# alpa-projects/alpa

Hardware: AMD Instinct MI355X
Metric: model_tflops_aggregate (higher is better)
Workload: dtype bf16; 1 GPU; model=GPT-2.6B, hidden=2560, layers=32, heads=32, vocab=51200, global_batch=32, seq_len=1024, num_micro_batches=1, parallelism=dp1, hip_graph=True

## Files before the change

alpa_amd/ops/__init__.py:

```python
from __future__ import annotations

import functools
import math
from typing import List, NamedTuple, Optional

import torch

from . import reference as ref
from ._backend import hip_ops, hip_ops_available, use_hip

__all__ = [
    "layer_norm", "add_layer_norm", "bias_gelu", "add_layer_norm_fp8",
    "bias_gelu_fp8", "flash_attention",
    "flash_attention_qkv", "flash_attention_decode", "decode_attn_ok",
    "DECODE_ATTN_CHUNK", "softmax_cross_entropy",
    "softmax_cross_entropy_partial", "softmax_cross_entropy_combine",
    "softmax_cross_entropy_shard_bwd", "vocab_ce_fused_ok", "fused_adamw",
    "multi_tensor_sumsq",
    "hip_ops_available", "MoERouting", "moe_top2_route", "moe_dispatch",
    "moe_combine", "moe_fused_ok",
]


class _LayerNorm(torch.autograd.Function):

    @staticmethod
    def forward(ctx, x, weight, bias, eps):
        x = x.contiguous()
        if use_hip(x):
            y, mean, rstd = hip_ops().layer_norm_fwd(x, weight, bias, eps)
        else:
            y, mean, rstd = ref.layer_norm_fwd(x, weight, bias, eps)
        ctx.save_for_backward(x, weight, mean, rstd)
        return y

    @staticmethod
    def backward(ctx, dy):
        x, weight, mean, rstd = ctx.saved_tensors
        if use_hip(x):
            dx, dw, db = hip_ops().layer_norm_bwd(dy.contiguous(), x, weight,
                                                  mean, rstd)
        else:
            dx, dw, db = ref.layer_norm_bwd(dy, x, weight, mean, rstd)
        return dx, dw.to(weight.dtype), db.to(weight.dtype), None


def layer_norm(x: torch.Tensor, weight: torch.Tensor, bias: torch.Tensor,
               eps: float = 1e-5) -> torch.Tensor:
    return _LayerNorm.apply(x, weight, bias, eps)


class _AddLayerNorm(torch.autograd.Function):

    @staticmethod
    def forward(ctx, a, delta, weight, bias, eps):
        a = a.contiguous()
        delta = delta.contiguous() if delta is not None else None
        if use_hip(a):
            h, y, mean, rstd = hip_ops().add_layer_norm_fwd(
                a, delta, weight, bias, eps)
        else:
            h = a + delta if delta is not None else a
            y, mean, rstd = ref.layer_norm_fwd(h, weight, bias, eps)
        ctx.save_for_backward(h, weight, mean, rstd)
        ctx.has_delta = delta is not None
        return h, y

    @staticmethod
    def backward(ctx, dh, dy):
        h, weight, mean, rstd = ctx.saved_tensors
        dy = dy.contiguous()
        dhc = dh.contiguous() if dh is not None else None
        if use_hip(h):
            dx, dw, db = hip_ops().add_layer_norm_bwd(dy, dhc, h, weight,
                                                      mean, rstd)
        else:
            dx, dw, db = ref.layer_norm_bwd(dy, h, weight, mean, rstd)
            if dhc is not None:
                dx = dx + dhc
        g2 = dx if ctx.has_delta else None
        return dx, g2, dw.to(weight.dtype), db.to(weight.dtype), None


def add_layer_norm(a: torch.Tensor, delta, weight: torch.Tensor,
                   bias: torch.Tensor, eps: float = 1e-5):
    if delta is None:
        return a, _LayerNorm.apply(a, weight, bias, eps)
    return _AddLayerNorm.apply(a, delta, weight, bias, eps)


class _BiasGelu(torch.autograd.Function):

    @staticmethod
    def forward(ctx, x, bias):
        x = x.contiguous()
        ctx.save_for_backward(x, bias)
        if use_hip(x):
            return hip_ops().bias_gelu_fwd(x, bias)
        return ref.bias_gelu_fwd(x, bias)

    @staticmethod
    def backward(ctx, dy):
        x, bias = ctx.saved_tensors
        if use_hip(x):
            dx, db = hip_ops().bias_gelu_bwd(dy.contiguous(), x, bias)
        else:
            dx, db = ref.bias_gelu_bwd(dy, x, bias)
        return dx, db.to(bias.dtype)


def bias_gelu(x: torch.Tensor, bias: torch.Tensor) -> torch.Tensor:
    return _BiasGelu.apply(x, bias)


@torch.no_grad()
def bias_gelu_fp8(x: torch.Tensor, bias: torch.Tensor, scale: torch.Tensor):
    x = x.contiguous()
    if use_hip(x):
        return tuple(hip_ops().bias_gelu_fp8(x, bias, scale))
    return ref.bias_gelu_fp8(x, bias, scale)


ADD_LAYER_NORM_FP8_MAX_H = 4096


@torch.no_grad()
def add_layer_norm_fp8(a: torch.Tensor, delta, weight: torch.Tensor,
                       bias: torch.Tensor, eps: float, scale: torch.Tensor):
    a = a.contiguous()
    delta = delta.contiguous() if delta is not None else None
    if use_hip(a):
        return tuple(hip_ops().add_layer_norm_fp8(a, delta, weight, bias,
                                                  eps, scale))
    return ref.add_layer_norm_fp8(a, delta, weight, bias, eps, scale)


class _BiasAdd(torch.autograd.Function):

    @staticmethod
    def forward(ctx, x, bias):
        ctx.feat = bias.shape[-1]
        ctx.bias_dtype = bias.dtype
        return x + bias

    @staticmethod
    def backward(ctx, g):
        if use_hip(g) and g.dtype == torch.bfloat16:
            db = hip_ops().colsum_bf16(
                g.contiguous().reshape(-1, ctx.feat))
            db = db.to(ctx.bias_dtype)
        else:
            dims = tuple(range(g.dim() - 1))
            db = g.sum(dim=dims).to(ctx.bias_dtype)
        return g, db


def bias_add(x: torch.Tensor, bias: torch.Tensor) -> torch.Tensor:
    return _BiasAdd.apply(x, bias)


class _LinearBias(torch.autograd.Function):

    @staticmethod
    def forward(ctx, x, w, bias):
        shape = x.shape
        x2 = x.reshape(-1, shape[-1])
        y = torch.addmm(bias, x2, w.t())
        ctx.save_for_backward(x2, w)
        ctx.bias_dtype = bias.dtype
        return y.reshape(*shape[:-1], w.shape[0])

    @staticmethod
    def backward(ctx, g):
        x2, w = ctx.saved_tensors
        g2 = g.reshape(-1, g.shape[-1]).contiguous()
        dx = (g2 @ w).reshape(*g.shape[:-1], w.shape[1])
        dw = g2.t() @ x2
        if use_hip(g2) and g2.dtype == torch.bfloat16:
            db = hip_ops().colsum_bf16(g2).to(ctx.bias_dtype)
        else:
            db = g2.sum(0).to(ctx.bias_dtype)
        return dx, dw, db


def linear_bias(x: torch.Tensor, w: torch.Tensor,
                bias: torch.Tensor) -> torch.Tensor:
    return _LinearBias.apply(x, w, bias)


class _FlashAttention(torch.autograd.Function):

    @staticmethod
    def forward(ctx, q, k, v, causal, scale, alibi=None):
        if scale is None:
            scale = 1.0 / math.sqrt(q.shape[-1])
        if use_hip(q):
            if q.shape[-1] > 128:
                assert alibi is None, "alibi requires head_dim <= 128"
                if q.shape[2] >= 128 and q.shape[-1] <= 256:
                    o, lse = hip_ops().attn_fwd(q, k, v, causal, scale,
                                                None)
                else:
                    o, lse = hip_ops().attn_fwd_blocked(q, k, v, causal,
                                                        scale)
            else:
                o, lse = hip_ops().attn_fwd(q, k, v, causal, scale, alibi)
        else:
            o, lse = ref.attention_fwd(q, k, v, causal, scale, alibi)
        ctx.save_for_backward(q, k, v, o, lse)
        ctx.causal = causal
        ctx.scale = scale
        ctx.alibi = alibi
        return o

    @staticmethod
    def backward(ctx, do):
        q, k, v, o, lse = ctx.saved_tensors
        if use_hip(q):
            if q.shape[-1] > 128:
                dq, dk, dv = hip_ops().attn_bwd_blocked(
                    do.contiguous(), q, k, v, o, lse, ctx.causal, ctx.scale)
            else:
                dq, dk, dv = hip_ops().attn_bwd(
                    do.contiguous(), q, k, v, o, lse, ctx.causal, ctx.scale,
                    ctx.alibi)
        else:
            dq, dk, dv = ref.attention_bwd(do, q, k, v, o, lse, ctx.causal,
                                           ctx.scale, ctx.alibi)
        return dq, dk, dv, None, None, None


def flash_attention(q: torch.Tensor, k: torch.Tensor, v: torch.Tensor,
                    causal: bool = True,
                    scale: Optional[float] = None,
                    alibi_slopes: Optional[torch.Tensor] = None
                    ) -> torch.Tensor:
    if q.shape[2] == 1 and not causal and _decode_attn_routed(q, k, v) and \
            not (torch.is_grad_enabled() and
                 (q.requires_grad or k.requires_grad or v.requires_grad)):
        if scale is None:
            scale = 1.0 / math.sqrt(q.shape[-1])
        return hip_ops().attn_decode(q, k, v, scale, alibi_slopes, None)[0]
    return _FlashAttention.apply(q, k, v, causal, scale, alibi_slopes)


_DECODE_ATTN_CHUNK = {64: 128, 128: 128, 256: 128}


def DECODE_ATTN_CHUNK(head_dim: int) -> int:
    for dp in sorted(_DECODE_ATTN_CHUNK):
        if head_dim <= dp:
            return _DECODE_ATTN_CHUNK[dp]
    raise ValueError(f"head_dim {head_dim} is above 256")


def _rows_aligned16(t: torch.Tensor) -> bool:
    return t.data_ptr() % 16 == 0 and all(
        t.shape[i] <= 1 or t.stride(i) % 8 == 0 for i in range(3))


def decode_attn_ok(q: torch.Tensor, k: torch.Tensor, v: torch.Tensor) -> bool:
    for t in (q, k, v):
        if not (t.is_cuda and t.dtype == torch.bfloat16 and t.dim() == 4
                and t.stride(3) == 1):
            return False
    D = q.shape[3]
    if q.shape[2] != 1 or D % 16 != 0 or not 16 <= D <= 256:
        return False
    if k.shape != v.shape or k.shape[:2] != q.shape[:2] or k.shape[3] != D \
            or q.shape[0] * q.shape[1] > 65535:
        return False
    if not all(_rows_aligned16(t) for t in (q, k, v)):
        return False
    return use_hip(q)


def _decode_attn_routed(q, k, v) -> bool:
    from ..global_env import global_config
    if global_config.decode_attention in ("0", False):
        return False
    return decode_attn_ok(q, k, v)


@torch.no_grad()
def flash_attention_decode(q: torch.Tensor, k: torch.Tensor, v: torch.Tensor,
                           kv_lens: Optional[torch.Tensor] = None,
                           scale: Optional[float] = None,
                           alibi_slopes: Optional[torch.Tensor] = None
                           ) -> torch.Tensor:
    if scale is None:
        scale = 1.0 / math.sqrt(q.shape[-1])
    lens = None if kv_lens is None else kv_lens.to(dtype=torch.int32)
    if decode_attn_ok(q, k, v):
        return hip_ops().attn_decode(
            q, k, v, scale, alibi_slopes,
            None if lens is None else lens.contiguous())[0]
    o, _ = ref.attention_fwd(q, k, v, False, scale, alibi_slopes, lens)
    return o


@torch.no_grad()
def flash_attention_varlen(q: torch.Tensor, k: torch.Tensor,
                           v: torch.Tensor, kv_lens: torch.Tensor,
                           scale: Optional[float] = None,
                           alibi_slopes: Optional[torch.Tensor] = None
                           ) -> torch.Tensor:
    if scale is None:
        scale = 1.0 / math.sqrt(q.shape[-1])
    lens = kv_lens.to(dtype=torch.int32)
    if use_hip(q):
        if q.shape[2] == 1 and _decode_attn_routed(q, k, v):
            return hip_ops().attn_decode(q, k, v, scale, alibi_slopes,
                                         lens.contiguous())[0]
        if q.shape[-1] > 128:
            raise NotImplementedError(
                "varlen attention with more than one query row, or with "
                "the decode kernel off, requires head_dim <= 128")
        o, _ = hip_ops().attn_fwd(q.contiguous(), k.contiguous(),
                                  v.contiguous(), False, scale,
                                  alibi_slopes, lens.contiguous())
        return o
    o, _ = ref.attention_fwd(q, k, v, False, scale, alibi_slopes, lens)
    return o


def _qkv_views(qkv: torch.Tensor, num_heads: int):
    B, S, F = qkv.shape
    qkv5 = qkv.view(B, S, num_heads, 3, F // (3 * num_heads))
    return tuple(qkv5[:, :, :, i].permute(0, 2, 1, 3) for i in range(3))


class _FlashAttentionQKV(torch.autograd.Function):

    @staticmethod
    def forward(ctx, qkv, num_heads, causal, scale):
        B, S, F = qkv.shape
        h = num_heads
        d = F // (3 * h)
        if scale is None:
            scale = 1.0 / math.sqrt(d)
        q, k, v = _qkv_views(qkv, h)
        if use_hip(qkv):
            o_buf = torch.empty(B, S, h * d, dtype=qkv.dtype,
                                device=qkv.device)
            o_view = o_buf.view(B, S, h, d).permute(0, 2, 1, 3)
            lse = torch.empty(B, h, S, dtype=torch.float32,
                              device=qkv.device)
            hip_ops().attn_fwd_out(q, k, v, o_view, lse, causal, scale)
        else:
            o4, lse = ref.attention_fwd(q.contiguous(), k.contiguous(),
                                        v.contiguous(), causal, scale)
            o_buf = o4.permute(0, 2, 1, 3).reshape(B, S, h * d)
        ctx.save_for_backward(qkv, o_buf, lse)
        ctx.meta = (num_heads, causal, scale)
        return o_buf

    @staticmethod
    def backward(ctx, do):
        qkv, o_buf, lse = ctx.saved_tensors
        h, causal, scale = ctx.meta
        B, S, F = qkv.shape
        d = F // (3 * h)
        q, k, v = _qkv_views(qkv, h)
        do4 = do.view(B, S, h, d).permute(0, 2, 1, 3)
        o4 = o_buf.view(B, S, h, d).permute(0, 2, 1, 3)
        dqkv = torch.empty_like(qkv)
        dq_v, dk_v, dv_v = _qkv_views(dqkv, h)
        if use_hip(qkv):
            hip_ops().attn_bwd_out(do4, q, k, v, o4, lse, dq_v, dk_v, dv_v,
                                   causal, scale)
        else:
            dq, dk, dv = ref.attention_bwd(
                do4.contiguous(), q.contiguous(), k.contiguous(),
                v.contiguous(), o4.contiguous(), lse, causal, scale)
            dq_v.copy_(dq)
            dk_v.copy_(dk)
            dv_v.copy_(dv)
        return dqkv, None, None, None


def flash_attention_qkv(qkv: torch.Tensor, num_heads: int,
                        causal: bool = True,
                        scale: Optional[float] = None) -> torch.Tensor:
    return _FlashAttentionQKV.apply(qkv, num_heads, causal, scale)


class _SoftmaxCrossEntropy(torch.autograd.Function):

    @staticmethod
    def forward(ctx, logits, targets):
        logits = logits.contiguous()
        if use_hip(logits):
            loss, lse = hip_ops().cross_entropy_fwd(logits, targets)
        else:
            loss, lse = ref.softmax_cross_entropy_fwd(logits, targets)
        ctx.save_for_backward(logits, targets, lse)
        return loss

    @staticmethod
    def backward(ctx, dloss):
        logits, targets, lse = ctx.saved_tensors
        if use_hip(logits):
            dlogits = hip_ops().cross_entropy_bwd(dloss.contiguous(), logits,
                                                  targets, lse)
        else:
            dlogits = ref.softmax_cross_entropy_bwd(dloss, logits, targets, lse)
        return dlogits, None


def softmax_cross_entropy(logits: torch.Tensor,
                          targets: torch.Tensor) -> torch.Tensor:
    return _SoftmaxCrossEntropy.apply(logits, targets)




def vocab_ce_fused_ok(logits: torch.Tensor) -> bool:
    if not (logits.is_cuda and logits.dtype == torch.bfloat16):
        return False
    if logits.dim() != 2 or not logits.is_contiguous():
        return False
    if logits.shape[-1] < 8 or logits.shape[-1] % 8 != 0 or \
            logits.data_ptr() % 16 != 0:
        return False
    return use_hip(logits)


@torch.no_grad()
def softmax_cross_entropy_partial(logits: torch.Tensor,
                                  targets: torch.Tensor,
                                  vocab_start: int) -> torch.Tensor:
    if use_hip(logits):
        return hip_ops().cross_entropy_partial_fwd(
            logits.contiguous(), targets.contiguous(), int(vocab_start))
    return ref.softmax_cross_entropy_partial(logits, targets,
                                             int(vocab_start))


@torch.no_grad()
def softmax_cross_entropy_combine(stats: torch.Tensor):
    return ref.softmax_cross_entropy_combine(stats)


@torch.no_grad()
def softmax_cross_entropy_shard_bwd(dloss: torch.Tensor,
                                    logits: torch.Tensor,
                                    targets: torch.Tensor, lse: torch.Tensor,
                                    vocab_start: int) -> torch.Tensor:
    if use_hip(logits):
        return hip_ops().cross_entropy_shard_bwd(
            dloss.contiguous(), logits.contiguous(), targets.contiguous(),
            lse, int(vocab_start))
    return ref.softmax_cross_entropy_shard_bwd(dloss, logits, targets, lse,
                                               int(vocab_start))


_ADAM_CHUNK = 16384
_ADAM_TABLE_CACHE: dict = {}


def _upload_tables(rows, dev):
    n = len(rows)
    descs = torch.tensor(rows, dtype=torch.int64).reshape(n, 6)
    counts = [(r[4] + _ADAM_CHUNK - 1) // _ADAM_CHUNK for r in rows]
    tensor_idx = torch.repeat_interleave(
        torch.arange(n, dtype=torch.int32),
        torch.tensor(counts, dtype=torch.int64))
    chunk_idx = torch.cat([torch.arange(c, dtype=torch.int32)
                           for c in counts])
    chunks = torch.stack([tensor_idx, chunk_idx], dim=1).contiguous()
    return descs.to(dev), chunks.to(dev)


def _adam_tables(params, grads, exp_avgs, exp_avg_sqs):
    key = tuple((p.data_ptr(), g.data_ptr(), m.data_ptr(), v.data_ptr(),
                 p.numel(), p.dtype)
                for p, g, m, v in zip(params, grads, exp_avgs, exp_avg_sqs))
    hit = _ADAM_TABLE_CACHE.get(key)
    if hit is not None:
        return hit
    rows = []
    for p, g, m, v in zip(params, grads, exp_avgs, exp_avg_sqs):
        assert p.is_contiguous() and g.is_contiguous()
        assert m.dtype == torch.float32 and v.dtype == torch.float32
        assert p.dtype == g.dtype and p.dtype in (torch.bfloat16,
                                                  torch.float32)
        rows.append((p.data_ptr(), g.data_ptr(), m.data_ptr(), v.data_ptr(),
                     p.numel(), 1 if p.dtype == torch.bfloat16 else 0))
    tbl = _upload_tables(rows, params[0].device)
    _ADAM_TABLE_CACHE[key] = tbl
    return tbl


_SUMSQ_TABLE_CACHE: dict = {}


def _sumsq_tables(tensors):
    key = tuple((t.data_ptr(), t.numel(), t.dtype) for t in tensors)
    hit = _SUMSQ_TABLE_CACHE.get(key)
    if hit is not None:
        return hit
    rows = []
    for t in tensors:
        assert t.is_contiguous()
        assert t.dtype in (torch.bfloat16, torch.float32)
        rows.append((0, t.data_ptr(), 0, 0, t.numel(),
                     1 if t.dtype == torch.bfloat16 else 0))
    dev = tensors[0].device
    descs, chunks = _upload_tables(rows, dev)
    partials = torch.empty(chunks.shape[0], dtype=torch.float32, device=dev)
    tbl = (descs, chunks, partials)
    _SUMSQ_TABLE_CACHE[key] = tbl
    return tbl


@torch.no_grad()
def multi_tensor_sumsq(tensors: List[torch.Tensor]) -> torch.Tensor:
    tensors = [t for t in tensors if t.numel() > 0]
    if not tensors:
        raise ValueError("multi_tensor_sumsq needs at least one element")
    if use_hip(tensors[0]):
        descs, chunks, partials = _sumsq_tables(tensors)
        out = torch.empty(1, dtype=torch.float32, device=tensors[0].device)
        hip_ops().multi_tensor_sumsq_raw(descs, chunks, partials, out)
        return out
    return ref.multi_tensor_sumsq(tensors)


@torch.no_grad()
def fused_adamw(params: List[torch.Tensor], grads: List[torch.Tensor],
                exp_avgs: List[torch.Tensor], exp_avg_sqs: List[torch.Tensor],
                step: int, lr: float, beta1: float = 0.9, beta2: float = 0.95,
                eps: float = 1e-8, weight_decay: float = 0.0,
                grad_scale: float = 1.0,
                grad_sumsq: Optional[torch.Tensor] = None,
                max_grad_norm: Optional[float] = None) -> None:
    if (grad_sumsq is None) != (max_grad_norm is None):
        raise ValueError(
            "grad_sumsq and max_grad_norm must be given together")
    if max_grad_norm is not None and not max_grad_norm > 0:
        raise ValueError(f"max_grad_norm must be > 0, got {max_grad_norm}")
    if not params:
        return
    if use_hip(params[0]):
        descs, chunks = _adam_tables(params, grads, exp_avgs, exp_avg_sqs)
        hip_ops().adamw_step_raw(descs, chunks, step, lr, beta1, beta2, eps,
                                 weight_decay, grad_scale, grad_sumsq,
                                 max_grad_norm or 0.0)
    else:
        ref.adamw_step(params, grads, exp_avgs, exp_avg_sqs, step, lr, beta1,
                       beta2, eps, weight_decay, grad_scale, grad_sumsq,
                       max_grad_norm)




class MoERouting(NamedTuple):
    w1: torch.Tensor
    w2: torch.Tensor
    idx1: torch.Tensor
    idx2: torch.Tensor
    slot1: torch.Tensor
    slot2: torch.Tensor
    src: torch.Tensor
    aux_loss: torch.Tensor


class _MoeTop2Route(torch.autograd.Function):

    @staticmethod
    def forward(ctx, logits, capacity):
        logits = logits.contiguous()
        if use_hip(logits):
            outs = hip_ops().moe_route_fwd(logits, capacity)
        else:
            outs = ref.moe_top2_route(logits, capacity)
        w1, w2, idx1, idx2, slot1, slot2, src, aux, count1 = outs
        ctx.save_for_backward(logits, idx1, idx2, w1, w2, count1)
        ctx.mark_non_differentiable(idx1, idx2, slot1, slot2, src)
        return w1, w2, idx1, idx2, slot1, slot2, src, aux

    @staticmethod
    def backward(ctx, dw1, dw2, _i1, _i2, _s1, _s2, _src, daux):
        logits, idx1, idx2, w1, w2, count1 = ctx.saved_tensors
        if use_hip(logits):
            return hip_ops().moe_route_bwd(
                logits, idx1, idx2, w1, w2, count1, dw1.float().contiguous(),
                dw2.float().contiguous(), daux.float().contiguous()), None
        return ref.moe_top2_route_bwd(logits, idx1, idx2, w1, w2, count1,
                                      dw1, dw2, daux), None


def moe_top2_route(logits: torch.Tensor, capacity: int) -> MoERouting:
    return MoERouting(*_MoeTop2Route.apply(logits, int(capacity)))


class _MoeDispatch(torch.autograd.Function):

    @staticmethod
    def forward(ctx, x, src, slot1, slot2):
        x = x.contiguous()
        ctx.save_for_backward(slot1, slot2)
        if use_hip(x):
            return hip_ops().moe_dispatch(x, src)
        return ref.moe_dispatch(x, src)

    @staticmethod
    def backward(ctx, g):
        slot1, slot2 = ctx.saved_tensors
        if use_hip(g):
            dx = hip_ops().moe_combine(g.contiguous(), None, None, slot1,
                                       slot2)
        else:
            dx = ref.moe_dispatch_bwd(g, slot1, slot2)
        return dx, None, None, None


def moe_dispatch(x: torch.Tensor, routing: MoERouting) -> torch.Tensor:
    return _MoeDispatch.apply(x, routing.src, routing.slot1, routing.slot2)


class _MoeCombine(torch.autograd.Function):

    @staticmethod
    def forward(ctx, y, w1, w2, slot1, slot2, src):
        y = y.contiguous()
        ctx.save_for_backward(y, w1, w2, slot1, slot2, src)
        if use_hip(y):
            return hip_ops().moe_combine(y, w1.float().contiguous(),
                                         w2.float().contiguous(), slot1,
                                         slot2)
        return ref.moe_combine(y, w1, w2, slot1, slot2)

    @staticmethod
    def backward(ctx, dout):
        y, w1, w2, slot1, slot2, src = ctx.saved_tensors
        if use_hip(y):
            dout = dout.contiguous()
            dy = hip_ops().moe_dispatch(dout, src, slot1,
                                        w1.float().contiguous(),
                                        w2.float().contiguous())
            dw1, dw2 = hip_ops().moe_combine_dw(dout, y, slot1, slot2)
            dw1, dw2 = dw1.to(w1.dtype), dw2.to(w2.dtype)
        else:
            dy, dw1, dw2 = ref.moe_combine_bwd(dout, y, w1, w2, slot1,
                                               slot2, src)
        return dy, dw1, dw2, None, None, None


def moe_combine(y: torch.Tensor, routing: MoERouting) -> torch.Tensor:
    return _MoeCombine.apply(y, routing.w1, routing.w2, routing.slot1,
                             routing.slot2, routing.src)


def moe_fused_ok(x: torch.Tensor, num_experts: int,
                 capacity: Optional[int] = None) -> bool:
    if not (x.is_cuda and x.dtype == torch.bfloat16):
        return False
    if x.shape[-1] < 8 or x.shape[-1] % 8 != 0 or \
            not 2 <= num_experts <= 128:
        return False
    if capacity is not None and num_experts * capacity >= 2 ** 31:
        return False
    return use_hip(x)



def _skinny_mt(M: int) -> int:
    MT = 4
    while MT < M:
        MT *= 2
    return MT


def _skinny_legal_splits(K: int, MT: int) -> List[int]:
    q = K // 64
    return [s for s in range(1, q + 1)
            if q % s == 0 and (K // 8 // s) * 16 * MT <= 65536]


@functools.lru_cache(maxsize=None)
def _skinny_splits(N: int, K: int, M: int) -> Optional[int]:
    lds_ok = _skinny_legal_splits(K, _skinny_mt(M))
    if not lds_ok:
        return None
    for s in sorted(lds_ok, reverse=True):
        if K // 8 // s >= 16 and (N // 64) * s >= 1024:
            return s
    for s in lds_ok:
        if (N // 64) * s >= 2560:
            return s
    return lds_ok[-1]


def _skinny_cache(module, weight: torch.Tensor, fp8: bool):
    key = (weight._version, fp8)
    cached = getattr(module, "_skinny_pack", None)
    if cached is not None and cached[0] == key:
        return cached[1], cached[2]
    N, K = weight.shape
    with torch.no_grad():
        w = weight.contiguous()
        if fp8:
            amax = w.abs().amax().float().clamp_min(1e-12)
            scale = (amax / 448.0).reshape(1)
            q = (w.float() / scale).clamp(-448.0, 448.0).to(
                torch.float8_e4m3fn)
            wp = q.view(torch.uint8).view(N, K // 8, 8) \
                .permute(1, 0, 2).contiguous()
        else:
            scale = None
            wp = w.view(N, K // 8, 8).permute(1, 0, 2).contiguous()
    module._skinny_pack = (key, wp, scale)
    return wp, scale


def skinny_ok(x: torch.Tensor, weight: torch.Tensor, module=None) -> bool:
    from ..global_env import global_config
    mode = global_config.skinny_gemm
    if mode in ("0", False) or torch.is_grad_enabled():
        return False
    if not (x.is_cuda and x.dtype == torch.bfloat16):
        return False
    if torch.cuda.is_current_stream_capturing() and \
            getattr(module, "_skinny_pack", None) is None:
        return False
    N, K = weight.shape
    if mode == "auto" and (K > 6144 and N > 6144):
        fp8 = (global_config.fp8_gemm and
               not getattr(module, "_fp8_exclude", False))
        if not fp8:
            return False
    m = x.numel() // x.shape[-1]
    return (m <= 8 and N % 64 == 0 and K % 64 == 0
            and _skinny_splits(N, K, m) is not None)


_SKINNY_TUNED = {}


def _skinny_tune(wp, x2, scale, N, K, MT):
    key = (N, K, MT, scale is not None)
    got = _SKINNY_TUNED.get(key)
    if got is not None:
        return got
    legal = _skinny_legal_splits(K, MT)
    cands = sorted({
        s for s in (
            next((c for c in reversed(legal)
                  if K // 8 // c >= 16 and (N // 64) * c >= 1024), None),
            next((c for c in legal if (N // 64) * c >= 2560), None),
            next((c for c in legal if K // 8 // c <= 32), None),
            legal[-1]) if s is not None})
    if len(cands) == 1:
        _SKINNY_TUNED[key] = cands[0]
        return cands[0]
    best, best_t = cands[0], float("inf")
    for c in cands:
        hip_ops().skinny_gemm(wp, x2, scale, None, N, K, c)
        t0 = torch.cuda.Event(True)
        t1 = torch.cuda.Event(True)
        t0.record()
        for _ in range(10):
            hip_ops().skinny_gemm(wp, x2, scale, None, N, K, c)
        t1.record()
        t1.synchronize()
        dt = t0.elapsed_time(t1)
        if dt < best_t:
            best, best_t = c, dt
    _SKINNY_TUNED[key] = best
    return best


def skinny_linear(x: torch.Tensor, weight: torch.Tensor,
                  bias: Optional[torch.Tensor], module) -> torch.Tensor:
    from ..global_env import global_config
    fp8 = (global_config.fp8_gemm and
           not getattr(module, "_fp8_exclude", False))
    wp, scale = _skinny_cache(module, weight, fp8)
    N, K = weight.shape
    shape = x.shape
    x2 = x.reshape(-1, K).contiguous()
    b = bias.contiguous() if bias is not None else None
    MT = _skinny_mt(x2.shape[0])
    if torch.cuda.is_current_stream_capturing():
        splits = _SKINNY_TUNED.get((N, K, MT, scale is not None)) \
            or _skinny_splits(N, K, x2.shape[0])
    else:
        splits = _skinny_tune(wp, x2, scale, N, K, MT)
    y = hip_ops().skinny_gemm(wp, x2, scale, b, N, K, splits)
    return y.reshape(*shape[:-1], N)
```

alpa_amd/ops/csrc/bias_gelu.hip:

```cpp
#include "common.h"
#include "fused_math.h"
#include "launchers.h"

__device__ __forceinline__ float gelu_grad_f(float x) {
  const float k = 0.7978845608028654f;
  float x2 = x * x;
  float sg = gelu_sigmoid(x);
  return sg + 2.0f * x * sg * (1.0f - sg) * k *
                  (1.0f + 3.f * 0.044715f * x2);
}

__global__ void bias_gelu_fwd_kernel(const short* __restrict__ x,
                                     const short* __restrict__ bias,
                                     short* __restrict__ y, int64_t total,
                                     int F) {
  int64_t idx = ((int64_t)blockIdx.x * blockDim.x + threadIdx.x) * 8;
  int64_t stride = (int64_t)gridDim.x * blockDim.x * 8;
  for (; idx < total; idx += stride) {
    bf16x8 v = *reinterpret_cast<const bf16x8*>(x + idx);
    bf16x8 bv = *reinterpret_cast<const bf16x8*>(bias + (idx % F));
    bf16x8 o;
#pragma unroll
    for (int j = 0; j < 8; ++j) o[j] = f2bf(gelu_f(bf2f(v[j]) + bf2f(bv[j])));
    *reinterpret_cast<bf16x8*>(y + idx) = o;
  }
}

__global__ void bias_gelu_bwd_dx_kernel(const short* __restrict__ dy,
                                        const short* __restrict__ x,
                                        const short* __restrict__ bias,
                                        short* __restrict__ dx, int64_t total,
                                        int F) {
  int64_t idx = ((int64_t)blockIdx.x * blockDim.x + threadIdx.x) * 8;
  int64_t stride = (int64_t)gridDim.x * blockDim.x * 8;
  for (; idx < total; idx += stride) {
    bf16x8 dv = *reinterpret_cast<const bf16x8*>(dy + idx);
    bf16x8 xv = *reinterpret_cast<const bf16x8*>(x + idx);
    bf16x8 bv = *reinterpret_cast<const bf16x8*>(bias + (idx % F));
    bf16x8 o;
#pragma unroll
    for (int j = 0; j < 8; ++j) {
      float z = bf2f(xv[j]) + bf2f(bv[j]);
      o[j] = f2bf(bf2f(dv[j]) * gelu_grad_f(z));
    }
    *reinterpret_cast<bf16x8*>(dx + idx) = o;
  }
}

__global__ void bias_grad_partial_kernel(const short* __restrict__ dx,
                                         float* __restrict__ part, int64_t N,
                                         int F) {
  const int col8 = (blockIdx.x * blockDim.x + threadIdx.x) * 8;
  const int p = blockIdx.y;
  const int P = gridDim.y;
  const int64_t r0 = (int64_t)p * N / P, r1 = (int64_t)(p + 1) * N / P;
  if (col8 + 8 <= F) {
    float s[8] = {0.f, 0.f, 0.f, 0.f, 0.f, 0.f, 0.f, 0.f};
    for (int64_t row = r0; row < r1; ++row) {
      bf16x8 v = *reinterpret_cast<const bf16x8*>(dx + row * F + col8);
#pragma unroll
      for (int j = 0; j < 8; ++j) s[j] += bf2f(v[j]);
    }
#pragma unroll
    for (int j = 0; j < 8; ++j) part[(int64_t)p * F + col8 + j] = s[j];
  } else if (col8 < F) {
    for (int c = col8; c < F; ++c) {
      float s = 0.f;
      for (int64_t row = r0; row < r1; ++row) s += bf2f(dx[row * F + c]);
      part[(int64_t)p * F + c] = s;
    }
  }
}

extern "C" {

hipError_t launch_bias_gelu_fwd(const void* x, const void* bias, void* y,
                                int64_t N, int64_t F, hipStream_t stream) {
  int64_t total = N * F;
  int blocks = (int)min((int64_t)2048, ceil_div(total, 256 * 8));
  bias_gelu_fwd_kernel<<<dim3(blocks), dim3(256), 0, stream>>>(
      (const short*)x, (const short*)bias, (short*)y, total, (int)F);
  return hipGetLastError();
}

hipError_t launch_colsum_partial(const void* t, float* part, int64_t N,
                                 int64_t F, int P, hipStream_t stream) {
  dim3 grid((uint32_t)ceil_div(F, 256 * 8), P);
  bias_grad_partial_kernel<<<grid, dim3(256), 0, stream>>>(
      (const short*)t, part, N, (int)F);
  return hipGetLastError();
}

hipError_t launch_bias_gelu_bwd(const void* dy, const void* x,
                                const void* bias, void* dx, float* db_part,
                                int64_t N, int64_t F, int P,
                                hipStream_t stream) {
  int64_t total = N * F;
  int blocks = (int)min((int64_t)2048, ceil_div(total, 256 * 8));
  bias_gelu_bwd_dx_kernel<<<dim3(blocks), dim3(256), 0, stream>>>(
      (const short*)dy, (const short*)x, (const short*)bias, (short*)dx,
      total, (int)F);
  dim3 grid((uint32_t)ceil_div(F, 256 * 8), P);
  bias_grad_partial_kernel<<<grid, dim3(256), 0, stream>>>(
      (const short*)dx, db_part, N, (int)F);
  return hipGetLastError();
}

}
```

alpa_amd/ops/csrc/bindings.cpp:

```cpp
#include <torch/extension.h>

#include <ATen/ATen.h>
#include <c10/hip/HIPStream.h>
#include <hip/hip_runtime.h>

#include <vector>
#include <algorithm>
#include <array>
#include <utility>

#include "launchers.h"

#define HIP_OK(expr)                                                       \
  do {                                                                     \
    hipError_t _e = (expr);                                                \
    TORCH_CHECK(_e == hipSuccess, "HIP error: ", hipGetErrorString(_e));   \
  } while (0)

namespace {

hipStream_t cur_stream() {
  return c10::hip::getCurrentHIPStream().stream();
}


const char* dtype_name(at::ScalarType dtype) {
  switch (dtype) {
    case at::kBFloat16: return "bf16";
    case at::kFloat: return "fp32";
    case at::kInt: return "int32";
    case at::kLong: return "int64";
    default: return c10::toString(dtype);
  }
}

void check_device(const at::Tensor& t, const char* name,
                  const at::Tensor& first) {
  TORCH_CHECK(t.is_cuda(), name, " must be on GPU");
  TORCH_CHECK(t.device() == first.device(), name, " is on ", t.device(),
              " but the first operand is on ", first.device());
}

void check_typed(const at::Tensor& t, const char* name, at::ScalarType dtype,
                 const at::Tensor& first) {
  check_device(t, name, first);
  TORCH_CHECK(t.scalar_type() == dtype, name, " must be ", dtype_name(dtype));
}

void check_vec(const at::Tensor& t, const char* name, at::ScalarType dtype,
               int64_t n, const at::Tensor& first) {
  check_typed(t, name, dtype, first);
  TORCH_CHECK(t.is_contiguous(), name, " must be contiguous");
  TORCH_CHECK(t.numel() == n, name, " must have ", n, " elements, got ",
              t.numel());
}

std::pair<int64_t, int64_t> check_rows(const at::Tensor& t, const char* name,
                                       int64_t m, const at::Tensor& first) {
  check_typed(t, name, at::kBFloat16, first);
  TORCH_CHECK(t.is_contiguous(), name, " must be contiguous");
  TORCH_CHECK(t.dim() >= 1, name, " must have a feature dimension");
  const int64_t W = t.size(-1);
  TORCH_CHECK(W > 0 && W % m == 0, name,
              ": the last dimension must be a positive multiple of ", m,
              ", got ", W);
  return {t.numel() / W, W};
}

void check_like(const at::Tensor& t, const char* name, const at::Tensor& ref,
                const char* ref_name) {
  check_typed(t, name, at::kBFloat16, ref);
  TORCH_CHECK(t.is_contiguous(), name, " must be contiguous");
  TORCH_CHECK(t.sizes() == ref.sizes(), name, " must have the shape of ",
              ref_name);
}

void check_bhsd(const at::Tensor& t, const char* name, int64_t B, int64_t H,
                int64_t S, int64_t D, const at::Tensor& first) {
  check_typed(t, name, at::kBFloat16, first);
  TORCH_CHECK(t.dim() == 4, name, " must be 4-D [B,H,S,D]");
  TORCH_CHECK(t.stride(3) == 1, name, " head-dim must be contiguous");
  const int64_t want[4] = {B, H, S, D};
  for (int i = 0; i < 4; ++i)
    TORCH_CHECK(want[i] < 0 || t.size(i) == want[i], name, " must have size ",
                want[i], " in dimension ", i, ", got ", t.size(i));
}

void check_rows_aligned16(const at::Tensor& t, const char* name) {
  TORCH_CHECK(reinterpret_cast<uintptr_t>(t.const_data_ptr()) % 16 == 0, name,
              " must be 16-byte aligned");
  for (int i = 0; i < 3; ++i)
    TORCH_CHECK(t.size(i) <= 1 || t.stride(i) % 8 == 0, name,
                ": the stride of dimension ", i,
                " must be a multiple of 8 elements, got ", t.stride(i));
}

std::pair<int64_t, int64_t> check_aligned_rows(const at::Tensor& t,
                                               const char* name,
                                               const at::Tensor& first) {
  auto dims = check_rows(t, name, 8, first);
  TORCH_CHECK(t.dim() == 2, name, " must be 2-D");
  TORCH_CHECK(reinterpret_cast<uintptr_t>(t.const_data_ptr()) % 16 == 0, name,
              " must be 16-byte aligned");
  return dims;
}

int stripes_for(int64_t N, int64_t cols, int64_t chunk_cols) {
  int64_t chunks = std::max<int64_t>(1, cols / chunk_cols);
  int64_t p = std::max<int64_t>(64, 2048 / chunks);
  return (int)std::min<int64_t>({p, N, 512});
}


std::vector<at::Tensor> layer_norm_fwd(const at::Tensor& x,
                                       const at::Tensor& w,
                                       const at::Tensor& b, double eps) {
  auto [N, H] = check_rows(x, "x", 8, x);
  check_vec(w, "w", at::kBFloat16, H, x);
  check_vec(b, "b", at::kBFloat16, H, x);
  auto y = at::empty_like(x);
  auto f32 = x.options().dtype(at::kFloat);
  auto mean = at::empty({N}, f32);
  auto rstd = at::empty({N}, f32);
  HIP_OK(launch_layer_norm_fwd(x.const_data_ptr(), w.const_data_ptr(),
                               b.const_data_ptr(), y.mutable_data_ptr(),
                               (float*)mean.mutable_data_ptr(),
                               (float*)rstd.mutable_data_ptr(), N, H,
                               (float)eps, cur_stream()));
  return {y, mean, rstd};
}

std::pair<at::Tensor, at::Tensor> layer_norm_dwdb(const at::Tensor& dy,
                                                  const at::Tensor& x,
                                                  const at::Tensor& mean,
                                                  const at::Tensor& rstd,
                                                  int64_t N, int64_t H) {
  auto f32 = x.options().dtype(at::kFloat);
  auto dw = at::empty({H}, f32);
  auto db = at::empty({H}, f32);
  const int kStripes = stripes_for(N, H, 256);
  auto dw_part = at::empty({kStripes, H}, f32);
  auto db_part = at::empty({kStripes, H}, f32);
  HIP_OK(launch_layer_norm_bwd_dwdb(
      dy.const_data_ptr(), x.const_data_ptr(),
      (const float*)mean.const_data_ptr(),
      (const float*)rstd.const_data_ptr(),
      (float*)dw_part.mutable_data_ptr(), (float*)db_part.mutable_data_ptr(),
      N, H, kStripes, cur_stream()));
  at::sum_out(dw, dw_part, {0});
  at::sum_out(db, db_part, {0});
  return {dw, db};
}

std::vector<at::Tensor> layer_norm_bwd(const at::Tensor& dy,
                                       const at::Tensor& x,
                                       const at::Tensor& w,
                                       const at::Tensor& mean,
                                       const at::Tensor& rstd) {
  auto [N, H] = check_rows(x, "x", 8, x);
  check_like(dy, "dy", x, "x");
  check_vec(w, "w", at::kBFloat16, H, x);
  check_vec(mean, "mean", at::kFloat, N, x);
  check_vec(rstd, "rstd", at::kFloat, N, x);
  auto dx = at::empty_like(x);
  HIP_OK(launch_layer_norm_bwd_dx(
      dy.const_data_ptr(), nullptr, x.const_data_ptr(), w.const_data_ptr(),
      (const float*)mean.const_data_ptr(), (const float*)rstd.const_data_ptr(),
      dx.mutable_data_ptr(), N, H, cur_stream()));
  auto [dw, db] = layer_norm_dwdb(dy, x, mean, rstd, N, H);
  return {dx, dw, db};
}


std::vector<at::Tensor> add_layer_norm_fwd(const at::Tensor& a,
                                           const c10::optional<at::Tensor>& b,
                                           const at::Tensor& w,
                                           const at::Tensor& bias,
                                           double eps) {
  auto [N, H] = check_rows(a, "a", 8, a);
  if (b.has_value()) check_like(*b, "b", a, "a");
  check_vec(w, "w", at::kBFloat16, H, a);
  check_vec(bias, "bias", at::kBFloat16, H, a);
  auto h = at::empty_like(a);
  auto y = at::empty_like(a);
  auto f32 = a.options().dtype(at::kFloat);
  auto mean = at::empty({N}, f32);
  auto rstd = at::empty({N}, f32);
  const void* bp = b.has_value() ? b->const_data_ptr() : nullptr;
  HIP_OK(launch_add_layer_norm_fwd(
      a.const_data_ptr(), bp, w.const_data_ptr(), bias.const_data_ptr(),
      h.mutable_data_ptr(), y.mutable_data_ptr(),
      (float*)mean.mutable_data_ptr(), (float*)rstd.mutable_data_ptr(), N,
      H, (float)eps, cur_stream()));
  return {h, y, mean, rstd};
}

std::vector<at::Tensor> add_layer_norm_bwd(
    const at::Tensor& dy, const c10::optional<at::Tensor>& dh,
    const at::Tensor& h, const at::Tensor& w, const at::Tensor& mean,
    const at::Tensor& rstd) {
  auto [N, H] = check_rows(h, "h", 8, h);
  check_like(dy, "dy", h, "h");
  if (dh.has_value()) check_like(*dh, "dh", h, "h");
  check_vec(w, "w", at::kBFloat16, H, h);
  check_vec(mean, "mean", at::kFloat, N, h);
  check_vec(rstd, "rstd", at::kFloat, N, h);
  auto dx = at::empty_like(h);
  const void* dhp = dh.has_value() ? dh->const_data_ptr() : nullptr;
  HIP_OK(launch_layer_norm_bwd_dx(
      dy.const_data_ptr(), dhp, h.const_data_ptr(), w.const_data_ptr(),
      (const float*)mean.const_data_ptr(),
      (const float*)rstd.const_data_ptr(), dx.mutable_data_ptr(), N, H,
      cur_stream()));
  auto [dw, db] = layer_norm_dwdb(dy, h, mean, rstd, N, H);
  return {dx, dw, db};
}


at::Tensor bias_gelu_fwd(const at::Tensor& x, const at::Tensor& bias) {
  auto [N, F] = check_rows(x, "x", 8, x);
  check_vec(bias, "bias", at::kBFloat16, F, x);
  auto y = at::empty_like(x);
  HIP_OK(launch_bias_gelu_fwd(x.const_data_ptr(), bias.const_data_ptr(),
                              y.mutable_data_ptr(), N, F, cur_stream()));
  return y;
}

std::vector<at::Tensor> bias_gelu_bwd(const at::Tensor& dy,
                                      const at::Tensor& x,
                                      const at::Tensor& bias) {
  auto [N, F] = check_rows(x, "x", 8, x);
  check_like(dy, "dy", x, "x");
  check_vec(bias, "bias", at::kBFloat16, F, x);
  auto dx = at::empty_like(x);
  auto f32 = x.options().dtype(at::kFloat);
  const int kStripes = stripes_for(N, F, 2048);
  auto db = at::empty({F}, f32);
  auto db_part = at::empty({kStripes, F}, f32);
  HIP_OK(launch_bias_gelu_bwd(dy.const_data_ptr(), x.const_data_ptr(),
                              bias.const_data_ptr(), dx.mutable_data_ptr(),
                              (float*)db_part.mutable_data_ptr(), N, F,
                              kStripes, cur_stream()));
  at::sum_out(db, db_part, {0});
  return {dx, db};
}

at::Tensor colsum_bf16(const at::Tensor& t) {
  auto [N, F] = check_rows(t, "t", 1, t);
  auto f32 = t.options().dtype(at::kFloat);
  const int kStripes = stripes_for(N, F, 2048);
  auto part = at::empty({kStripes, F}, f32);
  auto out = at::empty({F}, f32);
  HIP_OK(launch_colsum_partial(t.const_data_ptr(),
                               (float*)part.mutable_data_ptr(), N, F,
                               kStripes, cur_stream()));
  at::sum_out(out, part, {0});
  return out;
}


at::Tensor skinny_gemm(const at::Tensor& wp, const at::Tensor& x,
                       const c10::optional<at::Tensor>& wscale,
                       const c10::optional<at::Tensor>& bias,
                       int64_t N, int64_t K, int64_t splits) {
  TORCH_CHECK(N > 0 && N % 64 == 0, "N must be a positive multiple of 64");
  TORCH_CHECK(K > 0 && K % 64 == 0, "K must be a positive multiple of 64");
  const bool fp8 = wscale.has_value();
  if (fp8) {
    check_device(wp, "wp", wp);
    TORCH_CHECK(wp.element_size() == 1,
                "wp must hold one-byte elements when wscale is given");
    TORCH_CHECK(wp.is_contiguous() && wp.numel() == N * K,
                "wp must be contiguous with N*K elements");
    check_vec(*wscale, "wscale", at::kFloat, 1, wp);
  } else {
    check_vec(wp, "wp", at::kBFloat16, N * K, wp);
  }
  if (bias.has_value()) check_vec(*bias, "bias", at::kBFloat16, N, wp);
  auto [M, Kx] = check_rows(x, "x", 64, wp);
  TORCH_CHECK(x.dim() == 2 && Kx == K, "x must be [M, K]");
  TORCH_CHECK(M >= 1 && M <= 64, "skinny path is for M <= 64");
  int64_t MT = 4;
  while (MT < M) MT *= 2;
  TORCH_CHECK(splits >= 1 && (K / 64) % splits == 0 &&
                  (K / 8 / splits) * 16 * MT <= 65536,
              "splits must divide K/64 and leave (K/8/splits)*16*MT <= 65536");
  at::Tensor xp = x;
  if (MT != M) {
    xp = at::zeros({MT, K}, x.options());
    xp.narrow(0, 0, M).copy_(x);
  }
  auto part = at::empty({splits, MT, N}, x.options().dtype(at::kFloat));
  auto y = at::empty({M, N}, x.options());
  HIP_OK(launch_skinny_gemm(
      wp.const_data_ptr(), xp.const_data_ptr(),
      (float*)part.mutable_data_ptr(),
      bias.has_value() ? bias->const_data_ptr() : nullptr,
      y.mutable_data_ptr(),
      fp8 ? (const float*)wscale->const_data_ptr() : nullptr, M, MT, N, K,
      (int)splits, fp8 ? 1 : 0, cur_stream()));
  return y;
}


void adamw_step_raw(const at::Tensor& descs, const at::Tensor& chunks,
                    int64_t step, double lr, double beta1, double beta2,
                    double eps, double weight_decay, double grad_scale,
                    const c10::optional<at::Tensor>& grad_sumsq,
                    double max_grad_norm) {
  TORCH_CHECK(descs.dim() == 2 && descs.size(1) == 6, "descs must be [n, 6]");
  TORCH_CHECK(chunks.dim() == 2 && chunks.size(1) == 2,
              "chunks must be [m, 2]");
  check_vec(descs, "descs", at::kLong, descs.numel(), descs);
  check_vec(chunks, "chunks", at::kInt, chunks.numel(), descs);
  const float* sumsq = nullptr;
  if (grad_sumsq.has_value()) {
    check_vec(*grad_sumsq, "grad_sumsq", at::kFloat, 1, descs);
    TORCH_CHECK(max_grad_norm > 0, "max_grad_norm must be positive");
    sumsq = (const float*)grad_sumsq->const_data_ptr();
  }
  HIP_OK(launch_adamw(descs.const_data_ptr(), chunks.const_data_ptr(),
                      (int)chunks.size(0), (float)lr, (float)beta1,
                      (float)beta2, (float)eps, (float)weight_decay,
                      (float)grad_scale, (int)step, sumsq,
                      (float)max_grad_norm, cur_stream()));
}

void multi_tensor_sumsq_raw(const at::Tensor& descs, const at::Tensor& chunks,
                            at::Tensor& partials, at::Tensor& out) {
  TORCH_CHECK(descs.dim() == 2 && descs.size(1) == 6, "descs must be [n, 6]");
  TORCH_CHECK(chunks.dim() == 2 && chunks.size(1) == 2,
              "chunks must be [m, 2]");
  check_vec(descs, "descs", at::kLong, descs.numel(), descs);
  check_vec(chunks, "chunks", at::kInt, chunks.numel(), descs);
  int64_t n = chunks.size(0);
  check_typed(partials, "partials", at::kFloat, descs);
  TORCH_CHECK(partials.is_contiguous() && partials.numel() >= n,
              "partials must be contiguous with at least num_chunks elements");
  check_vec(out, "out", at::kFloat, 1, descs);
  HIP_OK(launch_multi_tensor_sumsq(
      descs.const_data_ptr(), chunks.const_data_ptr(), (int)n,
      (float*)partials.mutable_data_ptr(), (float*)out.mutable_data_ptr(),
      cur_stream()));
}


std::vector<at::Tensor> cross_entropy_fwd(const at::Tensor& logits,
                                          const at::Tensor& targets) {
  auto [N, V] = check_rows(logits, "logits", 8, logits);
  check_vec(targets, "targets", at::kLong, N, logits);
  auto f32 = logits.options().dtype(at::kFloat);
  auto loss = at::empty({N}, f32);
  auto lse = at::empty({N}, f32);
  HIP_OK(launch_ce_fwd(logits.const_data_ptr(),
                       (const int64_t*)targets.const_data_ptr(),
                       (float*)loss.mutable_data_ptr(),
                       (float*)lse.mutable_data_ptr(), N, V, cur_stream()));
  return {loss, lse};
}

at::Tensor cross_entropy_bwd(const at::Tensor& dloss, const at::Tensor& logits,
                             const at::Tensor& targets,
                             const at::Tensor& lse) {
  auto [N, V] = check_rows(logits, "logits", 8, logits);
  check_vec(targets, "targets", at::kLong, N, logits);
  check_vec(lse, "lse", at::kFloat, N, logits);
  check_device(dloss, "dloss", logits);
  TORCH_CHECK(dloss.numel() == N, "dloss must have ", N, " elements, got ",
              dloss.numel());
  auto dlogits = at::empty_like(logits);
  auto dl = dloss.to(at::kFloat).contiguous();
  HIP_OK(launch_ce_bwd((const float*)dl.const_data_ptr(), logits.const_data_ptr(),
                       (const int64_t*)targets.const_data_ptr(),
                       (const float*)lse.const_data_ptr(),
                       dlogits.mutable_data_ptr(), N, V, 0, cur_stream()));
  return dlogits;
}

at::Tensor cross_entropy_partial_fwd(const at::Tensor& logits,
                                     const at::Tensor& targets,
                                     int64_t vocab_start) {
  auto [N, V] = check_aligned_rows(logits, "logits", logits);
  check_vec(targets, "targets", at::kLong, N, logits);
  TORCH_CHECK(vocab_start >= 0, "vocab_start must be >= 0");
  auto stats = at::empty({3, N}, logits.options().dtype(at::kFloat));
  HIP_OK(launch_ce_partial_fwd(logits.const_data_ptr(),
                               (const int64_t*)targets.const_data_ptr(),
                               (float*)stats.mutable_data_ptr(), N, V,
                               vocab_start, cur_stream()));
  return stats;
}

at::Tensor cross_entropy_shard_bwd(const at::Tensor& dloss,
                                   const at::Tensor& logits,
                                   const at::Tensor& targets,
                                   const at::Tensor& lse,
                                   int64_t vocab_start) {
  auto [N, V] = check_aligned_rows(logits, "logits", logits);
  check_vec(targets, "targets", at::kLong, N, logits);
  TORCH_CHECK(vocab_start >= 0, "vocab_start must be >= 0");
  check_vec(lse, "lse", at::kFloat, N, logits);
  check_device(dloss, "dloss", logits);
  TORCH_CHECK(dloss.numel() == N, "dloss must have ", N, " elements, got ",
              dloss.numel());
  auto dlogits = at::empty_like(logits);
  auto dl = dloss.to(at::kFloat).contiguous();
  HIP_OK(launch_ce_bwd((const float*)dl.const_data_ptr(),
                       logits.const_data_ptr(),
                       (const int64_t*)targets.const_data_ptr(),
                       (const float*)lse.const_data_ptr(),
                       dlogits.mutable_data_ptr(), N, V, vocab_start,
                       cur_stream()));
  return dlogits;
}



template <typename... T>
std::array<int64_t, 3 * sizeof...(T)> bhs_strides(const T&... t) {
  std::array<int64_t, 3 * sizeof...(T)> s;
  int64_t* p = s.data();
  ((*p++ = t.stride(0), *p++ = t.stride(1), *p++ = t.stride(2)), ...);
  return s;
}

bool given(const c10::optional<at::Tensor>& t) {
  return t.has_value() && t->defined();
}

const void* opt_ptr(const c10::optional<at::Tensor>& t) {
  return given(t) ? t->const_data_ptr() : nullptr;
}

void check_attn_inputs(const at::Tensor& q, const at::Tensor& k,
                       const at::Tensor& v,
                       const c10::optional<at::Tensor>& alibi,
                       const c10::optional<at::Tensor>& kv_lens,
                       int64_t max_D) {
  check_bhsd(q, "q", -1, -1, -1, -1, q);
  const int64_t B = q.size(0), H = q.size(1), D = q.size(3);
  check_bhsd(k, "k", B, H, -1, D, q);
  check_bhsd(v, "v", B, H, k.size(2), D, q);
  TORCH_CHECK(D > 0 && D % 16 == 0 && D <= max_D,
              "head_dim must be a multiple of 16 up to ", max_D, ", got ", D);
  TORCH_CHECK(D <= 128 || !(given(alibi) || given(kv_lens)),
              "alibi and kv_lens need head_dim <= 128, got ", D);
  if (given(alibi)) check_vec(*alibi, "alibi", at::kFloat, H, q);
  if (given(kv_lens)) check_vec(*kv_lens, "kv_lens", at::kInt, B, q);
}

at::Tensor attn_fwd_out(const at::Tensor& q, const at::Tensor& k,
                        const at::Tensor& v, at::Tensor o, at::Tensor lse,
                        bool causal, double scale,
                        const c10::optional<at::Tensor>& alibi =
                            c10::nullopt,
                        const c10::optional<at::Tensor>& kv_lens =
                            c10::nullopt) {
  check_attn_inputs(q, k, v, alibi, kv_lens, 256);
  int64_t B = q.size(0), H = q.size(1), S = q.size(2), D = q.size(3);
  int64_t Skv = k.size(2);
  check_bhsd(o, "o", B, H, S, D, q);
  check_vec(lse, "lse", at::kFloat, B * H * S, q);
  const auto strides = bhs_strides(q, k, v, o);
  HIP_OK(launch_attn_fwd(q.const_data_ptr(), k.const_data_ptr(),
                         v.const_data_ptr(), o.mutable_data_ptr(),
                         (float*)lse.mutable_data_ptr(), B, H, S, Skv, D,
                         (float)scale, causal ? 1 : 0,
                         (const float*)opt_ptr(alibi),
                         (const int*)opt_ptr(kv_lens), strides.data(),
                         cur_stream()));
  return o;
}

std::vector<at::Tensor> attn_fwd(const at::Tensor& q, const at::Tensor& k,
                                 const at::Tensor& v, bool causal,
                                 double scale,
                                 const c10::optional<at::Tensor>& alibi =
                                     c10::nullopt,
                                 const c10::optional<at::Tensor>& kv_lens =
                                     c10::nullopt) {
  check_attn_inputs(q, k, v, alibi, kv_lens, 256);
  int64_t B = q.size(0), H = q.size(1), S = q.size(2);
  auto o = at::empty_like(q.contiguous());
  auto lse = at::empty({B, H, S}, q.options().dtype(at::kFloat));
  attn_fwd_out(q, k, v, o, lse, causal, scale, alibi, kv_lens);
  return {o, lse};
}

std::vector<at::Tensor> attn_decode(const at::Tensor& q, const at::Tensor& k,
                                    const at::Tensor& v, double scale,
                                    const c10::optional<at::Tensor>& alibi =
                                        c10::nullopt,
                                    const c10::optional<at::Tensor>& kv_lens =
                                        c10::nullopt) {
  check_bhsd(q, "q", -1, -1, -1, -1, q);
  const int64_t B = q.size(0), H = q.size(1), D = q.size(3);
  TORCH_CHECK(q.size(2) == 1, "q must hold one query row per head, got ",
              q.size(2));
  check_bhsd(k, "k", B, H, -1, D, q);
  const int64_t Skv = k.size(2);
  check_bhsd(v, "v", B, H, Skv, D, q);
  TORCH_CHECK(D > 0 && D % 16 == 0 && D <= 256,
              "head_dim must be a multiple of 16 up to 256, got ", D);
  TORCH_CHECK(B * H <= 65535, "q: at most 65535 (batch, head) pairs, got ",
              B * H);
  if (given(alibi)) check_vec(*alibi, "alibi", at::kFloat, H, q);
  if (given(kv_lens)) check_vec(*kv_lens, "kv_lens", at::kInt, B, q);
  check_rows_aligned16(q, "q");
  check_rows_aligned16(k, "k");
  check_rows_aligned16(v, "v");
  auto f32 = q.options().dtype(at::kFloat);
  auto o = at::empty({B, H, 1, D}, q.options());
  auto lse = at::empty({B, H, 1}, f32);
  if (B * H == 0) return {o, lse};
  auto ws = at::empty({attn_decode_workspace_floats(B, H, Skv, D)}, f32);
  const auto strides = bhs_strides(q, k, v, o);
  HIP_OK(launch_attn_decode(q.const_data_ptr(), k.const_data_ptr(),
                            v.const_data_ptr(), o.mutable_data_ptr(),
                            (float*)lse.mutable_data_ptr(),
                            (float*)ws.mutable_data_ptr(), B, H, Skv, D,
                            (float)scale, (const float*)opt_ptr(alibi),
                            (const int*)opt_ptr(kv_lens), strides.data(),
                            cur_stream()));
  return {o, lse};
}

std::vector<at::Tensor> attn_fwd_blocked(const at::Tensor& q_,
                                         const at::Tensor& k_,
                                         const at::Tensor& v_, bool causal,
                                         double scale) {
  auto q = q_.contiguous(), k = k_.contiguous(), v = v_.contiguous();
  int64_t B = q.size(0), H = q.size(1), S = q.size(2);
  int64_t Skv = k.size(2);
  auto o = at::empty_like(q);
  auto lse = at::empty({B, H, S}, q.options().dtype(at::kFloat));
  const int64_t BQ = 256;
  int64_t qoff = Skv - S;
  for (int64_t qs = 0; qs < S; qs += BQ) {
    int64_t qe = std::min(qs + BQ, S);
    auto qb = q.slice(2, qs, qe);
    int64_t ke = causal ? std::min(qe + qoff, Skv) : Skv;
    auto kb = k.slice(2, 0, ke);
    auto s_blk = at::matmul(qb, kb.transpose(-1, -2)).to(at::kFloat)
                     .mul_(scale);
    if (causal) {
      auto qi = at::arange(qs + qoff, qe + qoff, q.options().dtype(at::kLong));
      auto kj = at::arange(ke, q.options().dtype(at::kLong));
      auto mask = kj.view({1, 1, 1, ke}) > qi.view({1, 1, qe - qs, 1});
      s_blk.masked_fill_(mask, -std::numeric_limits<float>::infinity());
    }
    auto m = std::get<0>(s_blk.max(-1, true));
    auto p = at::exp(s_blk - m);
    auto l = p.sum(-1, true);
    o.slice(2, qs, qe).copy_(
        at::matmul((p / l).to(at::kBFloat16), v.slice(2, 0, ke)));
    lse.slice(2, qs, qe).copy_((m + at::log(l)).squeeze(-1));
  }
  return {o, lse};
}

std::vector<at::Tensor> attn_bwd_blocked(const at::Tensor& dout_, const at::Tensor& q_,
                                 const at::Tensor& k_, const at::Tensor& v_,
                                 const at::Tensor& o_, const at::Tensor& lse,
                                 bool causal, double scale) {
  auto q = q_.contiguous(), k = k_.contiguous(), v = v_.contiguous();
  auto dout = dout_.contiguous(), o = o_.contiguous();
  int64_t B = q.size(0), H = q.size(1), S = q.size(2), D = q.size(3);
  int64_t Skv = k.size(2);
  auto dq = at::empty_like(q);
  auto dk = at::zeros_like(k, k.options().dtype(at::kFloat));
  auto dv = at::zeros_like(v, v.options().dtype(at::kFloat));
  auto delta = (dout.to(at::kFloat) * o.to(at::kFloat)).sum(-1, true);
  auto lse4 = lse.view({B, H, S, 1});
  const int64_t BQ = 256;
  for (int64_t qs = 0; qs < S; qs += BQ) {
    int64_t qe = std::min(qs + BQ, S);
    auto qb = q.slice(2, qs, qe);
    auto dob = dout.slice(2, qs, qe);
    int64_t ke = causal ? std::min(qe, Skv) : Skv;
    auto kb = k.slice(2, 0, ke);
    auto vb = v.slice(2, 0, ke);
    auto s = at::matmul(qb, kb.transpose(-1, -2));
    auto p = at::exp(s.to(at::kFloat) * scale - lse4.slice(2, qs, qe));
    if (causal) p = p.tril_(qs);
    auto p_bf = p.to(at::kBFloat16);
    dv.slice(2, 0, ke).add_(at::matmul(p_bf.transpose(-1, -2), dob));
    auto dp = at::matmul(dob, vb.transpose(-1, -2));
    auto ds = p.mul_(dp.to(at::kFloat) - delta.slice(2, qs, qe))
                  .mul_(scale);
    auto ds_bf = ds.to(at::kBFloat16);
    dq.slice(2, qs, qe).copy_(at::matmul(ds_bf, kb));
    dk.slice(2, 0, ke).add_(at::matmul(ds_bf.transpose(-1, -2), qb));
  }
  return {dq, dk.to(k.scalar_type()), dv.to(v.scalar_type())};
}

void check_attn_bwd_inputs(const at::Tensor& dout, const at::Tensor& q,
                           const at::Tensor& k, const at::Tensor& v,
                           const at::Tensor& o, const at::Tensor& lse,
                           const c10::optional<at::Tensor>& alibi) {
  check_attn_inputs(q, k, v, alibi, c10::nullopt, 128);
  const int64_t B = q.size(0), H = q.size(1), S = q.size(2), D = q.size(3);
  check_bhsd(dout, "dout", B, H, S, D, q);
  check_bhsd(o, "o", B, H, S, D, q);
  check_typed(lse, "lse", at::kFloat, q);
  TORCH_CHECK(lse.numel() == B * H * S, "lse must have ", B * H * S,
              " elements, got ", lse.numel());
}

void attn_bwd_out(const at::Tensor& dout, const at::Tensor& q,
                  const at::Tensor& k, const at::Tensor& v,
                  const at::Tensor& o, const at::Tensor& lse, at::Tensor dq,
                  at::Tensor dk, at::Tensor dv, bool causal, double scale,
                  const c10::optional<at::Tensor>& alibi = c10::nullopt) {
  check_attn_bwd_inputs(dout, q, k, v, o, lse, alibi);
  int64_t B = q.size(0), H = q.size(1), S = q.size(2), D = q.size(3);
  int64_t Skv = k.size(2);
  check_bhsd(dq, "dq", B, H, S, D, q);
  check_bhsd(dk, "dk", B, H, Skv, D, q);
  check_bhsd(dv, "dv", B, H, Skv, D, q);
  auto delta = at::empty({B, H, S}, q.options().dtype(at::kFloat));
  auto lse_c = lse.contiguous();
  const auto strides = bhs_strides(q, k, v, dout, dq, dk, dv, o);
  HIP_OK(launch_attn_bwd(q.const_data_ptr(), k.const_data_ptr(),
                         v.const_data_ptr(), o.const_data_ptr(),
                         dout.const_data_ptr(),
                         (const float*)lse_c.const_data_ptr(),
                         (float*)delta.mutable_data_ptr(),
                         dq.mutable_data_ptr(), dk.mutable_data_ptr(),
                         dv.mutable_data_ptr(), B, H, S, Skv, D,
                         (float)scale, causal ? 1 : 0,
                         (const float*)opt_ptr(alibi), strides.data(),
                         cur_stream()));
}

std::vector<at::Tensor> attn_bwd(const at::Tensor& dout, const at::Tensor& q,
                                 const at::Tensor& k, const at::Tensor& v,
                                 const at::Tensor& o, const at::Tensor& lse,
                                 bool causal, double scale,
                                 const c10::optional<at::Tensor>& alibi =
                                     c10::nullopt) {
  check_attn_bwd_inputs(dout, q, k, v, o, lse, alibi);
  auto dq = at::empty_like(q.contiguous());
  auto dk = at::empty_like(k.contiguous());
  auto dv = at::empty_like(v.contiguous());
  attn_bwd_out(dout, q, k, v, o, lse, dq, dk, dv, causal, scale, alibi);
  return {dq, dk, dv};
}


constexpr int64_t kMoeMaxTokens = int64_t(1) << 30;

std::vector<at::Tensor> moe_route_fwd(const at::Tensor& logits,
                                      int64_t capacity) {
  auto [N, E] = check_rows(logits, "logits", 1, logits);
  TORCH_CHECK(logits.dim() == 2, "logits must be [N, E]");
  const int64_t C = capacity;
  TORCH_CHECK(E >= 2 && E <= 128, "num_experts must be in [2, 128], got ", E);
  TORCH_CHECK(C >= 1, "capacity must be >= 1");
  TORCH_CHECK(C < (int64_t(1) << 31) / E, "E * capacity must be < 2^31");
  TORCH_CHECK(N <= kMoeMaxTokens, "at most 2^30 tokens");
  auto f32 = logits.options().dtype(at::kFloat);
  auto i32 = logits.options().dtype(at::kInt);
  auto w1 = at::empty({N}, f32), w2 = at::empty({N}, f32);
  auto idx1 = at::empty({N}, i32), idx2 = at::empty({N}, i32);
  auto slot1 = at::empty({N}, i32), slot2 = at::empty({N}, i32);
  if (N == 0) {
    return {w1, w2, idx1, idx2, slot1, slot2, at::full({E * C}, -1, i32),
            at::zeros({}, f32), at::zeros({E}, i32)};
  }
  auto src = at::empty({E * C}, i32);
  auto aux = at::empty({}, f32);
  auto count1 = at::empty({E}, i32);
  const int64_t nblocks = (N + 255) / 256;
  auto hist = at::empty({2, nblocks, E}, i32);
  auto ppart = at::empty({nblocks, E}, f32);
  auto psum = at::empty({E}, f32);
  int* hist1 = (int*)hist.mutable_data_ptr();
  int* hist2 = hist1 + nblocks * E;
  HIP_OK(launch_moe_route(
      logits.const_data_ptr(), (float*)w1.mutable_data_ptr(),
      (float*)w2.mutable_data_ptr(), (int*)idx1.mutable_data_ptr(),
      (int*)idx2.mutable_data_ptr(), (int*)slot1.mutable_data_ptr(),
      (int*)slot2.mutable_data_ptr(), hist1, hist2,
      (float*)ppart.mutable_data_ptr(), N, E, cur_stream()));
  at::sum_out(psum, ppart, {0});
  HIP_OK(launch_moe_slots(
      (const int*)idx1.const_data_ptr(), (const int*)idx2.const_data_ptr(),
      hist1, hist2, (const float*)psum.const_data_ptr(),
      (int*)count1.mutable_data_ptr(), (float*)aux.mutable_data_ptr(),
      (int*)slot1.mutable_data_ptr(), (int*)slot2.mutable_data_ptr(),
      (int*)src.mutable_data_ptr(), N, E, C, cur_stream()));
  return {w1, w2, idx1, idx2, slot1, slot2, src, aux, count1};
}

at::Tensor moe_route_bwd(const at::Tensor& logits, const at::Tensor& idx1,
                         const at::Tensor& idx2, const at::Tensor& w1,
                         const at::Tensor& w2, const at::Tensor& count1,
                         const at::Tensor& dw1, const at::Tensor& dw2,
                         const at::Tensor& daux) {
  auto [N, E] = check_rows(logits, "logits", 1, logits);
  TORCH_CHECK(logits.dim() == 2, "logits must be [N, E]");
  TORCH_CHECK(E >= 2 && E <= 128, "num_experts must be in [2, 128], got ", E);
  TORCH_CHECK(N <= kMoeMaxTokens, "at most 2^30 tokens");
  check_vec(idx1, "idx1", at::kInt, N, logits);
  check_vec(idx2, "idx2", at::kInt, N, logits);
  check_vec(count1, "count1", at::kInt, E, logits);
  check_vec(w1, "w1", at::kFloat, N, logits);
  check_vec(w2, "w2", at::kFloat, N, logits);
  check_vec(dw1, "dw1", at::kFloat, N, logits);
  check_vec(dw2, "dw2", at::kFloat, N, logits);
  check_vec(daux, "daux", at::kFloat, 1, logits);
  auto dlogits = at::empty_like(logits);
  if (N == 0) return dlogits;
  HIP_OK(launch_moe_route_bwd(
      logits.const_data_ptr(), (const int*)idx1.const_data_ptr(),
      (const int*)idx2.const_data_ptr(), (const float*)w1.const_data_ptr(),
      (const float*)w2.const_data_ptr(), (const int*)count1.const_data_ptr(),
      (const float*)dw1.const_data_ptr(), (const float*)dw2.const_data_ptr(),
      (const float*)daux.const_data_ptr(), dlogits.mutable_data_ptr(), N, E,
      cur_stream()));
  return dlogits;
}

at::Tensor moe_dispatch(const at::Tensor& x, const at::Tensor& src,
                        const c10::optional<at::Tensor>& slot1,
                        const c10::optional<at::Tensor>& w1,
                        const c10::optional<at::Tensor>& w2) {
  auto [N, H] = check_aligned_rows(x, "x", x);
  const int64_t S = src.numel();
  check_vec(src, "src", at::kInt, S, x);
  TORCH_CHECK(S < (int64_t(1) << 31), "E * capacity must be < 2^31");
  TORCH_CHECK(N <= kMoeMaxTokens, "at most 2^30 tokens");
  const bool scaled = slot1.has_value();
  TORCH_CHECK(w1.has_value() == scaled && w2.has_value() == scaled,
              "slot1, w1 and w2 go together");
  if (scaled) {
    check_vec(*slot1, "slot1", at::kInt, N, x);
    check_vec(*w1, "w1", at::kFloat, N, x);
    check_vec(*w2, "w2", at::kFloat, N, x);
  }
  auto out = at::empty({S, H}, x.options());
  if (S == 0) return out;
  HIP_OK(launch_moe_dispatch(
      x.const_data_ptr(), (const int*)src.const_data_ptr(),
      scaled ? (const int*)slot1->const_data_ptr() : nullptr,
      scaled ? (const float*)w1->const_data_ptr() : nullptr,
      scaled ? (const float*)w2->const_data_ptr() : nullptr,
      out.mutable_data_ptr(), S, N, H, cur_stream()));
  return out;
}

at::Tensor moe_combine(const at::Tensor& y,
                       const c10::optional<at::Tensor>& w1,
                       const c10::optional<at::Tensor>& w2,
                       const at::Tensor& slot1, const at::Tensor& slot2) {
  auto [S, H] = check_aligned_rows(y, "y", y);
  const int64_t N = slot1.numel();
  TORCH_CHECK(S < (int64_t(1) << 31), "E * capacity must be < 2^31");
  TORCH_CHECK(N <= kMoeMaxTokens, "at most 2^30 tokens");
  check_vec(slot1, "slot1", at::kInt, N, y);
  check_vec(slot2, "slot2", at::kInt, N, y);
  TORCH_CHECK(w1.has_value() == w2.has_value(), "w1 and w2 go together");
  if (w1.has_value()) {
    check_vec(*w1, "w1", at::kFloat, N, y);
    check_vec(*w2, "w2", at::kFloat, N, y);
  }
  auto out = at::empty({N, H}, y.options());
  if (N == 0) return out;
  HIP_OK(launch_moe_combine(
      y.const_data_ptr(),
      w1.has_value() ? (const float*)w1->const_data_ptr() : nullptr,
      w2.has_value() ? (const float*)w2->const_data_ptr() : nullptr,
      (const int*)slot1.const_data_ptr(), (const int*)slot2.const_data_ptr(),
      out.mutable_data_ptr(), N, S, H, cur_stream()));
  return out;
}

std::vector<at::Tensor> moe_combine_dw(const at::Tensor& dout,
                                       const at::Tensor& y,
                                       const at::Tensor& slot1,
                                       const at::Tensor& slot2) {
  auto [N, H] = check_aligned_rows(dout, "dout", dout);
  auto [S, Hy] = check_aligned_rows(y, "y", dout);
  TORCH_CHECK(Hy == H, "dout and y must share H");
  TORCH_CHECK(S < (int64_t(1) << 31), "E * capacity must be < 2^31");
  TORCH_CHECK(N <= kMoeMaxTokens, "at most 2^30 tokens");
  check_vec(slot1, "slot1", at::kInt, N, dout);
  check_vec(slot2, "slot2", at::kInt, N, dout);
  auto f32 = dout.options().dtype(at::kFloat);
  auto dw1 = at::empty({N}, f32), dw2 = at::empty({N}, f32);
  if (N == 0) return {dw1, dw2};
  HIP_OK(launch_moe_combine_dw(
      dout.const_data_ptr(), y.const_data_ptr(),
      (const int*)slot1.const_data_ptr(), (const int*)slot2.const_data_ptr(),
      (float*)dw1.mutable_data_ptr(), (float*)dw2.mutable_data_ptr(), N, S,
      H, cur_stream()));
  return {dw1, dw2};
}

at::Tensor mfma_probe(const at::Tensor& a, const at::Tensor& b) {
  check_vec(a, "a", at::kBFloat16, 512, a);
  check_vec(b, "b", at::kBFloat16, 512, a);
  auto d = at::empty({16, 16}, a.options().dtype(at::kFloat));
  HIP_OK(launch_mfma_probe(a.const_data_ptr(), b.const_data_ptr(),
                           (float*)d.mutable_data_ptr(), cur_stream()));
  return d;
}

at::Tensor mfma_probe32(const at::Tensor& a, const at::Tensor& b) {
  check_vec(a, "a", at::kBFloat16, 512, a);
  check_vec(b, "b", at::kBFloat16, 512, a);
  auto d = at::empty({32, 32}, a.options().dtype(at::kFloat));
  HIP_OK(launch_mfma_probe32(a.const_data_ptr(), b.const_data_ptr(),
                             (float*)d.mutable_data_ptr(), cur_stream()));
  return d;
}

std::vector<at::Tensor> fp8_quantize(const at::Tensor& x,
                                     const at::Tensor& scale, bool dual,
                                     bool e5m2) {
  check_vec(x, "x", at::kBFloat16, x.numel(), x);
  check_vec(scale, "scale", at::kFloat, 1, x);
  auto qtype = e5m2 ? at::kFloat8_e5m2 : at::kFloat8_e4m3fn;
  auto amax = at::zeros({1}, x.options().dtype(at::kFloat));
  auto q = at::empty(x.sizes(), x.options().dtype(qtype));
  if (!dual) {
    TORCH_CHECK(x.numel() % 8 == 0, "numel must be divisible by 8");
    HIP_OK(launch_fp8_quantize(x.const_data_ptr(), q.data_ptr(),
                               (const float*)scale.const_data_ptr(),
                               (float*)amax.data_ptr(), x.numel(),
                               e5m2 ? 1 : 0, cur_stream()));
    return {q, at::Tensor(), amax};
  }
  TORCH_CHECK(x.dim() == 2, "dual quantize needs a 2-D tensor");
  int64_t M = x.size(0), N = x.size(1);
  auto qt = at::empty({N, M}, x.options().dtype(qtype));
  HIP_OK(launch_fp8_quantize_dual(x.const_data_ptr(), q.data_ptr(),
                                  qt.data_ptr(),
                                  (const float*)scale.const_data_ptr(),
                                  (float*)amax.data_ptr(), M, N,
                                  e5m2 ? 1 : 0, cur_stream()));
  return {q, qt, amax};
}


constexpr int64_t kFusedQuantMaxRows = int64_t(1) << 21;

std::vector<at::Tensor> bias_gelu_fp8(const at::Tensor& x,
                                      const at::Tensor& bias,
                                      const at::Tensor& scale) {
  auto [N, F] = check_rows(x, "x", 8, x);
  TORCH_CHECK(N < kFusedQuantMaxRows, "at most 2^21 rows");
  check_vec(bias, "bias", at::kBFloat16, F, x);
  check_vec(scale, "scale", at::kFloat, 1, x);
  auto q8 = x.options().dtype(at::kFloat8_e4m3fn);
  auto amax = at::zeros({1}, x.options().dtype(at::kFloat));
  auto q = at::empty({N, F}, q8);
  auto qt = at::empty({F, N}, q8);
  if (N == 0) return {q, qt, amax};
  HIP_OK(launch_bias_gelu_fp8(x.const_data_ptr(), bias.const_data_ptr(),
                              q.data_ptr(), qt.data_ptr(),
                              (const float*)scale.const_data_ptr(),
                              (float*)amax.data_ptr(), N, F, cur_stream()));
  return {q, qt, amax};
}

std::vector<at::Tensor> add_layer_norm_fp8(
    const at::Tensor& a, const c10::optional<at::Tensor>& b,
    const at::Tensor& w, const at::Tensor& bias, double eps,
    const at::Tensor& scale) {
  auto [N, H] = check_rows(a, "a", 8, a);
  TORCH_CHECK(H <= 4096, "add_layer_norm_fp8 handles H <= 4096, got ", H);
  TORCH_CHECK(N < kFusedQuantMaxRows, "at most 2^21 rows");
  if (b.has_value()) check_like(*b, "b", a, "a");
  check_vec(w, "w", at::kBFloat16, H, a);
  check_vec(bias, "bias", at::kBFloat16, H, a);
  check_vec(scale, "scale", at::kFloat, 1, a);
  auto f32 = a.options().dtype(at::kFloat);
  auto q8 = a.options().dtype(at::kFloat8_e4m3fn);
  auto h = at::empty_like(a);
  auto mean = at::empty({N}, f32);
  auto rstd = at::empty({N}, f32);
  auto amax = at::zeros({1}, f32);
  auto q = at::empty({N, H}, q8);
  auto qt = at::empty({H, N}, q8);
  if (N == 0) return {h, mean, rstd, q, qt, amax};
  const void* bp = b.has_value() ? b->const_data_ptr() : nullptr;
  HIP_OK(launch_add_layer_norm_fp8(
      a.const_data_ptr(), bp, w.const_data_ptr(), bias.const_data_ptr(),
      h.mutable_data_ptr(), q.data_ptr(), qt.data_ptr(),
      (float*)mean.mutable_data_ptr(), (float*)rstd.mutable_data_ptr(),
      (const float*)scale.const_data_ptr(), (float*)amax.data_ptr(), N, H,
      (float)eps, cur_stream()));
  return {h, mean, rstd, q, qt, amax};
}

}

PYBIND11_MODULE(TORCH_EXTENSION_NAME, m) {
  m.attr("ABI_VERSION") = 8;
  m.def("layer_norm_fwd", &layer_norm_fwd, "LayerNorm forward (gfx950)");
  m.def("layer_norm_bwd", &layer_norm_bwd, "LayerNorm backward (gfx950)");
  m.def("add_layer_norm_fwd", &add_layer_norm_fwd,
        "fused residual-add + LayerNorm fwd (gfx950)");
  m.def("add_layer_norm_bwd", &add_layer_norm_bwd,
        "fused residual-add + LayerNorm bwd (gfx950)");
  m.def("bias_gelu_fwd", &bias_gelu_fwd, "bias+GeLU forward (gfx950)");
  m.def("bias_gelu_bwd", &bias_gelu_bwd, "bias+GeLU backward (gfx950)");
  m.def("colsum_bf16", &colsum_bf16, "striped column sum (gfx950)");
  m.def("skinny_gemm", &skinny_gemm,
        "decode GEMV over packed weights (gfx950)");
  m.def("adamw_step_raw", &adamw_step_raw, "multi-tensor AdamW (gfx950)",
        py::arg("descs"), py::arg("chunks"), py::arg("step"), py::arg("lr"),
        py::arg("beta1"), py::arg("beta2"), py::arg("eps"),
        py::arg("weight_decay"), py::arg("grad_scale"),
        py::arg("grad_sumsq") = py::none(), py::arg("max_grad_norm") = 0.0);
  m.def("multi_tensor_sumsq_raw", &multi_tensor_sumsq_raw,
        "multi-tensor sum of squares (gfx950)");
  m.def("fp8_quantize", &fp8_quantize,
        "one-pass fp8 amax+cast, optional transposed twin (gfx950)");
  m.def("bias_gelu_fp8", &bias_gelu_fp8,
        "bias+GeLU forward emitting e4m3 q, qt and amax (gfx950)");
  m.def("add_layer_norm_fp8", &add_layer_norm_fp8,
        "residual-add + LayerNorm fwd emitting e4m3 q, qt and amax (gfx950)");
  m.def("cross_entropy_fwd", &cross_entropy_fwd, "fused CE fwd (gfx950)");
  m.def("cross_entropy_bwd", &cross_entropy_bwd, "fused CE bwd (gfx950)");
  m.def("cross_entropy_partial_fwd", &cross_entropy_partial_fwd,
        "vocab-shard CE partial stats [3, N] (gfx950)");
  m.def("cross_entropy_shard_bwd", &cross_entropy_shard_bwd,
        "vocab-shard CE bwd (gfx950)");
  m.def("attn_fwd", &attn_fwd, "flash attention fwd (gfx950 MFMA)",
        py::arg("q"), py::arg("k"), py::arg("v"), py::arg("causal"),
        py::arg("scale"), py::arg("alibi") = py::none(),
        py::arg("kv_lens") = py::none());
  m.def("attn_fwd_out", &attn_fwd_out, "flash attention fwd, strided out",
        py::arg("q"), py::arg("k"), py::arg("v"), py::arg("o"),
        py::arg("lse"), py::arg("causal"), py::arg("scale"),
        py::arg("alibi") = py::none(), py::arg("kv_lens") = py::none());
  m.def("attn_decode", &attn_decode,
        "split-KV decode attention, one query row per head (gfx950)",
        py::arg("q"), py::arg("k"), py::arg("v"), py::arg("scale"),
        py::arg("alibi") = py::none(), py::arg("kv_lens") = py::none());
  m.def("attn_decode_chunk",
        [](int64_t D) { return attn_decode_chunk(D); },
        "keys per split-KV chunk of attn_decode at head_dim D");
  m.def("attn_fwd_blocked", &attn_fwd_blocked,
        "blocked fwd for head_dim > 128 (hipBLASLt scores)");
  m.def("attn_bwd", &attn_bwd, "flash attention bwd (gfx950 MFMA)",
        py::arg("dout"), py::arg("q"), py::arg("k"), py::arg("v"),
        py::arg("o"), py::arg("lse"), py::arg("causal"), py::arg("scale"),
        py::arg("alibi") = py::none());
  m.def("attn_bwd_out", &attn_bwd_out, "flash attention bwd, strided out",
        py::arg("dout"), py::arg("q"), py::arg("k"), py::arg("v"),
        py::arg("o"), py::arg("lse"), py::arg("dq"), py::arg("dk"),
        py::arg("dv"), py::arg("causal"), py::arg("scale"),
        py::arg("alibi") = py::none());
  m.def("attn_bwd_blocked", &attn_bwd_blocked,
        "attention bwd (blocked hipBLASLt reference)");
  m.def("moe_route_fwd", &moe_route_fwd,
        "top-2 gate + capacity slots, sync-free (gfx950)");
  m.def("moe_route_bwd", &moe_route_bwd, "top-2 gate backward (gfx950)");
  m.def("moe_dispatch", &moe_dispatch, "MoE token dispatch gather (gfx950)",
        py::arg("x"), py::arg("src"), py::arg("slot1") = py::none(),
        py::arg("w1") = py::none(), py::arg("w2") = py::none());
  m.def("moe_combine", &moe_combine, "MoE weighted combine gather (gfx950)");
  m.def("moe_combine_dw", &moe_combine_dw,
        "MoE combine gate-weight gradient (gfx950)");
  m.def("mfma_probe", &mfma_probe, "MFMA 16x16x32 layout probe");
  m.def("mfma_probe32", &mfma_probe32, "MFMA 32x32x16 layout probe");
}
```

alpa_amd/ops/csrc/launchers.h:

```cpp
#pragma once

#include <hip/hip_runtime.h>

#include <cstdint>

extern "C" {

hipError_t launch_layer_norm_fwd(const void* x, const void* w, const void* b,
                                 void* y, float* mean, float* rstd, int64_t N,
                                 int64_t H, float eps, hipStream_t stream);
hipError_t launch_layer_norm_bwd_dx(const void* dy, const void* dh,
                                    const void* x, const void* w,
                                    const float* mean, const float* rstd,
                                    void* dx, int64_t N, int64_t H,
                                    hipStream_t stream);
hipError_t launch_layer_norm_bwd_dwdb(const void* dy, const void* x,
                                      const float* mean, const float* rstd,
                                      float* dw_part, float* db_part,
                                      int64_t N, int64_t H, int P,
                                      hipStream_t stream);
hipError_t launch_add_layer_norm_fwd(const void* a, const void* b,
                                     const void* w, const void* bias,
                                     void* h, void* y, float* mean,
                                     float* rstd, int64_t N, int64_t H,
                                     float eps, hipStream_t stream);

hipError_t launch_bias_gelu_fwd(const void* x, const void* bias, void* y,
                                int64_t N, int64_t F, hipStream_t stream);
hipError_t launch_bias_gelu_bwd(const void* dy, const void* x,
                                const void* bias, void* dx, float* db_part,
                                int64_t N, int64_t F, int P,
                                hipStream_t stream);
hipError_t launch_colsum_partial(const void* t, float* part, int64_t N,
                                 int64_t F, int P, hipStream_t stream);

hipError_t launch_adamw(const void* descs_dev, const void* chunks_dev,
                        int num_chunks, float lr, float beta1, float beta2,
                        float eps, float weight_decay, float grad_scale,
                        int step, const float* sumsq_or_null, float max_norm,
                        hipStream_t stream);
hipError_t launch_multi_tensor_sumsq(const void* descs_dev,
                                     const void* chunks_dev, int num_chunks,
                                     float* partials, float* sumsq,
                                     hipStream_t stream);

hipError_t launch_fp8_quantize(const void* src, void* q, const float* scale,
                               float* amax, int64_t total, int e5m2,
                               hipStream_t stream);
hipError_t launch_fp8_quantize_dual(const void* src, void* q, void* qt,
                                    const float* scale, float* amax,
                                    int64_t M, int64_t N, int e5m2,
                                    hipStream_t stream);

hipError_t launch_bias_gelu_fp8(const void* x, const void* bias, void* q,
                                void* qt, const float* scale, float* amax,
                                int64_t M, int64_t F, hipStream_t stream);
hipError_t launch_add_layer_norm_fp8(const void* a, const void* b,
                                     const void* w, const void* bias, void* h,
                                     void* q, void* qt, float* mean,
                                     float* rstd, const float* scale,
                                     float* amax, int64_t N, int64_t H,
                                     float eps, hipStream_t stream);

hipError_t launch_skinny_gemm(const void* wp, const void* x, float* part,
                              const void* bias_or_null, void* y,
                              const float* wscale_or_null, int64_t M,
                              int64_t MT, int64_t N, int64_t K, int splits,
                              int fp8, hipStream_t stream);

hipError_t launch_ce_fwd(const void* logits, const int64_t* targets,
                         float* loss, float* lse, int64_t N, int64_t V,
                         hipStream_t stream);
hipError_t launch_ce_partial_fwd(const void* logits, const int64_t* targets,
                                 float* stats, int64_t N, int64_t V,
                                 int64_t vocab_start, hipStream_t stream);
hipError_t launch_ce_bwd(const float* dloss, const void* logits,
                         const int64_t* targets, const float* lse,
                         void* dlogits, int64_t N, int64_t V,
                         int64_t vocab_start, hipStream_t stream);

hipError_t launch_attn_fwd(const void* q, const void* k, const void* v,
                           void* o, float* lse, int64_t B, int64_t H,
                           int64_t S, int64_t Skv, int64_t D, float scale,
                           int causal, const float* alibi,
                           const int* kv_lens, const int64_t* strides,
                           hipStream_t stream);
hipError_t launch_attn_bwd(const void* q, const void* k, const void* v,
                           const void* o, const void* dout,
                           const float* lse, float* delta_ws, void* dq,
                           void* dk, void* dv, int64_t B, int64_t H,
                           int64_t S, int64_t Skv, int64_t D, float scale,
                           int causal, const float* alibi,
                           const int64_t* strides, hipStream_t stream);

int attn_decode_chunk(int64_t D);
int64_t attn_decode_workspace_floats(int64_t B, int64_t H, int64_t Skv,
                                     int64_t D);
hipError_t launch_attn_decode(const void* q, const void* k, const void* v,
                              void* o, float* lse, float* ws, int64_t B,
                              int64_t H, int64_t Skv, int64_t D, float scale,
                              const float* alibi, const int* kv_lens,
                              const int64_t* strides, hipStream_t stream);

hipError_t launch_moe_route(const void* logits, float* w1, float* w2,
                            int* idx1, int* idx2, int* slot1, int* slot2,
                            int* hist1, int* hist2, float* ppart, int64_t N,
                            int64_t E, hipStream_t stream);
hipError_t launch_moe_slots(const int* idx1, const int* idx2, int* hist1,
                            int* hist2, const float* psum, int* count1,
                            float* aux, int* slot1, int* slot2, int* src,
                            int64_t N, int64_t E, int64_t C,
                            hipStream_t stream);
hipError_t launch_moe_route_bwd(const void* logits, const int* idx1,
                                const int* idx2, const float* w1,
                                const float* w2, const int* count1,
                                const float* dw1, const float* dw2,
                                const float* daux, void* dlogits, int64_t N,
                                int64_t E, hipStream_t stream);
hipError_t launch_moe_dispatch(const void* x, const int* src,
                               const int* slot1_or_null,
                               const float* w1_or_null,
                               const float* w2_or_null, void* out, int64_t S,
                               int64_t N, int64_t H, hipStream_t stream);
hipError_t launch_moe_combine(const void* y, const float* w1_or_null,
                              const float* w2_or_null, const int* slot1,
                              const int* slot2, void* out, int64_t N,
                              int64_t S, int64_t H, hipStream_t stream);
hipError_t launch_moe_combine_dw(const void* dout, const void* y,
                                 const int* slot1, const int* slot2,
                                 float* dw1, float* dw2, int64_t N, int64_t S,
                                 int64_t H, hipStream_t stream);

hipError_t launch_mfma_probe(const void* a, const void* b, float* d,
                             hipStream_t stream);
hipError_t launch_mfma_probe32(const void* a, const void* b, float* d,
                               hipStream_t stream);

}
```

alpa_amd/ops/csrc/layernorm.hip:

```cpp
#include "common.h"
#include "launchers.h"
#include "layernorm_rows.h"

__global__ void layer_norm_fwd_kernel(const short* __restrict__ x,
                                      const short* __restrict__ w,
                                      const short* __restrict__ b,
                                      short* __restrict__ y,
                                      float* __restrict__ mean_out,
                                      float* __restrict__ rstd_out,
                                      int H, float eps) {
  __shared__ float red[LN_BLOCK / 64];
  const int row = blockIdx.x;
  short* yr = y + (int64_t)row * H;
  layer_norm_rows<1, false>(
      x, nullptr, w, b, nullptr, mean_out, rstd_out, red, row, H, eps,
      [&](int, int i, bf16x8 o) { *reinterpret_cast<bf16x8*>(yr + i) = o; });
}

__global__ void add_layer_norm_fwd_kernel(const short* __restrict__ a,
                                          const short* __restrict__ b,
                                          const short* __restrict__ w,
                                          const short* __restrict__ bias,
                                          short* __restrict__ h,
                                          short* __restrict__ y,
                                          float* __restrict__ mean_out,
                                          float* __restrict__ rstd_out,
                                          int H, float eps) {
  __shared__ float red[LN_BLOCK / 64];
  const int row = blockIdx.x;
  short* yr = y + (int64_t)row * H;
  layer_norm_rows<1, true>(
      a, b, w, bias, h, mean_out, rstd_out, red, row, H, eps,
      [&](int, int i, bf16x8 o) { *reinterpret_cast<bf16x8*>(yr + i) = o; });
}

template <bool HAS_DH>
__global__ void layer_norm_bwd_dx_kernel(
    const short* __restrict__ dy, const short* __restrict__ dh,
    const short* __restrict__ x, const short* __restrict__ w,
    const float* __restrict__ mean_in, const float* __restrict__ rstd_in,
    short* __restrict__ dx, int H) {
  const int row = blockIdx.x;
  const short* dyr = dy + (int64_t)row * H;
  const short* dhr = HAS_DH ? dh + (int64_t)row * H : nullptr;
  const short* xr = x + (int64_t)row * H;
  short* dxr = dx + (int64_t)row * H;
  const float mean = mean_in[row], rstd = rstd_in[row];
  __shared__ float red[LN_BLOCK / 64];

  float c1 = 0.f, c2 = 0.f;
  for (int i = threadIdx.x * 8; i < H; i += LN_BLOCK * 8) {
    bf16x8 dv = *reinterpret_cast<const bf16x8*>(dyr + i);
    bf16x8 xv = *reinterpret_cast<const bf16x8*>(xr + i);
    bf16x8 wv = *reinterpret_cast<const bf16x8*>(w + i);
#pragma unroll
    for (int j = 0; j < 8; ++j) {
      float wdy = bf2f(dv[j]) * bf2f(wv[j]);
      float xhat = (bf2f(xv[j]) - mean) * rstd;
      c1 += wdy;
      c2 += wdy * xhat;
    }
  }
  c1 = block_reduce_sum(c1, red) / H;
  c2 = block_reduce_sum(c2, red) / H;

  for (int i = threadIdx.x * 8; i < H; i += LN_BLOCK * 8) {
    bf16x8 dv = *reinterpret_cast<const bf16x8*>(dyr + i);
    bf16x8 xv = *reinterpret_cast<const bf16x8*>(xr + i);
    bf16x8 wv = *reinterpret_cast<const bf16x8*>(w + i);
    bf16x8 hv;
    if (HAS_DH) hv = *reinterpret_cast<const bf16x8*>(dhr + i);
    bf16x8 o;
#pragma unroll
    for (int j = 0; j < 8; ++j) {
      float wdy = bf2f(dv[j]) * bf2f(wv[j]);
      float xhat = (bf2f(xv[j]) - mean) * rstd;
      float g = (wdy - c1 - xhat * c2) * rstd;
      if (HAS_DH) g += bf2f(hv[j]);
      o[j] = f2bf(g);
    }
    *reinterpret_cast<bf16x8*>(dxr + i) = o;
  }
}

#define LNB_COLS 256

__global__ void layer_norm_bwd_dwdb_partial(const short* __restrict__ dy,
                                            const short* __restrict__ x,
                                            const float* __restrict__ mean_in,
                                            const float* __restrict__ rstd_in,
                                            float* __restrict__ dw_part,
                                            float* __restrict__ db_part,
                                            int N, int H) {
  const int col4 = (blockIdx.x * LNB_COLS + threadIdx.x) * 4;
  const int p = blockIdx.y;
  const int P = gridDim.y;
  const int64_t r0 = (int64_t)p * N / P, r1 = (int64_t)(p + 1) * N / P;
  if (col4 + 4 <= H) {
    float dw[4] = {0.f, 0.f, 0.f, 0.f}, db[4] = {0.f, 0.f, 0.f, 0.f};
    for (int64_t row = r0; row < r1; ++row) {
      float mean = mean_in[row], rstd = rstd_in[row];
      bf16x4 dv = *reinterpret_cast<const bf16x4*>(dy + row * H + col4);
      bf16x4 xv = *reinterpret_cast<const bf16x4*>(x + row * H + col4);
#pragma unroll
      for (int j = 0; j < 4; ++j) {
        float d = bf2f(dv[j]);
        dw[j] += d * (bf2f(xv[j]) - mean) * rstd;
        db[j] += d;
      }
    }
#pragma unroll
    for (int j = 0; j < 4; ++j) {
      dw_part[(int64_t)p * H + col4 + j] = dw[j];
      db_part[(int64_t)p * H + col4 + j] = db[j];
    }
  } else if (col4 < H) {
    for (int c = col4; c < H; ++c) {
      float dw = 0.f, db = 0.f;
      for (int64_t row = r0; row < r1; ++row) {
        float mean = mean_in[row], rstd = rstd_in[row];
        float d = bf2f(dy[row * H + c]);
        dw += d * (bf2f(x[row * H + c]) - mean) * rstd;
        db += d;
      }
      dw_part[(int64_t)p * H + c] = dw;
      db_part[(int64_t)p * H + c] = db;
    }
  }
}

extern "C" {

hipError_t launch_layer_norm_fwd(const void* x, const void* w, const void* b,
                                 void* y, float* mean, float* rstd, int64_t N,
                                 int64_t H, float eps, hipStream_t stream) {
  layer_norm_fwd_kernel<<<dim3((uint32_t)N), dim3(LN_BLOCK), 0, stream>>>(
      (const short*)x, (const short*)w, (const short*)b, (short*)y, mean,
      rstd, (int)H, eps);
  return hipGetLastError();
}

hipError_t launch_layer_norm_bwd_dx(const void* dy, const void* dh,
                                    const void* x, const void* w,
                                    const float* mean, const float* rstd,
                                    void* dx, int64_t N, int64_t H,
                                    hipStream_t stream) {
  auto kernel = dh != nullptr ? layer_norm_bwd_dx_kernel<true>
                              : layer_norm_bwd_dx_kernel<false>;
  kernel<<<dim3((uint32_t)N), dim3(LN_BLOCK), 0, stream>>>(
      (const short*)dy, (const short*)dh, (const short*)x, (const short*)w,
      mean, rstd, (short*)dx, (int)H);
  return hipGetLastError();
}

hipError_t launch_layer_norm_bwd_dwdb(const void* dy, const void* x,
                                      const float* mean, const float* rstd,
                                      float* dw_part, float* db_part,
                                      int64_t N, int64_t H, int P,
                                      hipStream_t stream) {
  dim3 grid((uint32_t)ceil_div(H, LNB_COLS * 4), P);
  layer_norm_bwd_dwdb_partial<<<grid, dim3(LNB_COLS), 0, stream>>>(
      (const short*)dy, (const short*)x, mean, rstd, dw_part, db_part,
      (int)N, (int)H);
  return hipGetLastError();
}

hipError_t launch_add_layer_norm_fwd(const void* a, const void* b,
                                     const void* w, const void* bias,
                                     void* h, void* y, float* mean,
                                     float* rstd, int64_t N, int64_t H,
                                     float eps, hipStream_t stream) {
  add_layer_norm_fwd_kernel<<<dim3((uint32_t)N), dim3(LN_BLOCK), 0,
                              stream>>>(
      (const short*)a, (const short*)b, (const short*)w, (const short*)bias,
      (short*)h, (short*)y, mean, rstd, (int)H, eps);
  return hipGetLastError();
}

}
```

alpa_amd/ops/fp8.py:

```python
from __future__ import annotations

from typing import Optional

import torch

from ._backend import hip_ops

E4M3_MAX = 448.0
AMAX_DECAY = 0.999

_EPOCH = 0


def bump_epoch() -> None:
    global _EPOCH
    _EPOCH += 1


def fp8_available(x: torch.Tensor) -> bool:
    return (x.is_cuda and hasattr(torch, "float8_e4m3fn")
            and hasattr(torch, "_scaled_mm"))


class _RoleState:

    __slots__ = ("running", "scale")

    def __init__(self):
        self.running = None
        self.scale = None

    def ensure(self, ref: torch.Tensor):
        if self.scale is None:
            with torch.no_grad():
                amax = ref.abs().amax().float().clamp_min(1e-12).reshape(1)
                self.running = amax.clone()
                self.scale = (amax / E4M3_MAX).contiguous()

    @torch.no_grad()
    def update(self, amax: torch.Tensor):
        torch.maximum(amax, self.running * AMAX_DECAY, out=self.running)
        self.scale.copy_(self.running.clamp_min(1e-12) / E4M3_MAX)


def _role(module, name: str) -> _RoleState:
    st = getattr(module, f"_fp8_{name}", None)
    if st is None:
        st = _RoleState()
        setattr(module, f"_fp8_{name}", st)
    return st


def quantize(x2: torch.Tensor, state: _RoleState, dual: bool):
    state.ensure(x2)
    used = state.scale.clone()
    q, qt, amax = hip_ops().fp8_quantize(x2, used, dual, False)
    state.update(amax)
    return q, qt, used


def quantize_weight_cached(module, weight: torch.Tensor,
                           dual: bool = True):
    cached = getattr(module, "_fp8_cache", None)
    graphing = torch.cuda.is_current_stream_capturing() \
        if weight.is_cuda else False
    if cached is not None and cached[0] == _EPOCH and not graphing \
            and (not dual or cached[2] is not None):
        return cached[1], cached[2], cached[3]
    st = _role(module, "w")
    with torch.no_grad():
        wq, wqt, ws = quantize(weight.contiguous(), st, dual=dual)
    module._fp8_cache = (_EPOCH, wq, wqt, ws)
    return wq, wqt, ws


def _linear_fwd(ctx, xq, xqt, x_scale, x2, w, bias, module, infer,
                out_dtype):
    from ..global_env import global_config
    wgrad_fp8 = global_config.fp8_wgrad
    dx_bf16 = global_config.fp8_dx_bf16
    wq, wqt, ws = quantize_weight_cached(
        module, w, dual=(not dx_bf16) and not infer)
    y = torch._scaled_mm(xq, wq.t(), scale_a=x_scale, scale_b=ws,
                         bias=bias, out_dtype=out_dtype)
    if infer:
        return y, ()
    ctx.module = module
    ctx.wgrad_fp8 = wgrad_fp8
    ctx.dx_bf16 = dx_bf16
    ctx.has_bias = bias is not None
    wb = w if dx_bf16 else wqt
    return y, ((xqt if wgrad_fp8 else x2), wb, x_scale, ws)


def _linear_bwd(ctx, xsaved, wb, sx, ws, dy):
    module = ctx.module
    dy2 = dy.reshape(-1, dy.shape[-1]).contiguous()
    if ctx.wgrad_fp8 or not ctx.dx_bf16:
        sg = _role(module, "g")
        dyq, dyqt, g_scale = quantize(dy2, sg, dual=ctx.wgrad_fp8)
    if ctx.dx_bf16:
        dx = dy2 @ wb
    else:
        dx = torch._scaled_mm(dyq, wb.t(), scale_a=g_scale,
                              scale_b=ws, out_dtype=dy.dtype)
    if ctx.wgrad_fp8:
        dw = torch._scaled_mm(dyqt, xsaved.t(), scale_a=g_scale,
                              scale_b=sx, out_dtype=dy.dtype)
    else:
        dw = dy2.t() @ xsaved
    db = None
    if ctx.has_bias:
        db = hip_ops().colsum_bf16(dy2).to(dy.dtype)
    return dx, dw, db


class _Fp8Linear(torch.autograd.Function):

    @staticmethod
    def forward(ctx, x, w, bias, module, infer):
        from ..global_env import global_config
        shape = x.shape
        x2 = x.reshape(-1, shape[-1]).contiguous()
        sx = _role(module, "x")
        xq, xqt, x_scale = quantize(
            x2, sx, dual=global_config.fp8_wgrad and not infer)
        y, saved = _linear_fwd(ctx, xq, xqt, x_scale, x2, w, bias, module,
                               infer, x.dtype)
        if not infer:
            ctx.save_for_backward(*saved)
        return y.reshape(*shape[:-1], w.shape[0])

    @staticmethod
    def backward(ctx, dy):
        dx, dw, db = _linear_bwd(ctx, *ctx.saved_tensors, dy)
        return (dx.reshape(*dy.shape[:-1], dx.shape[-1]), dw, db, None, None)


def fp8_linear(x: torch.Tensor, weight: torch.Tensor,
               bias: Optional[torch.Tensor] = None,
               module=None) -> torch.Tensor:
    assert module is not None, "fp8_linear needs the owning module"
    infer = not torch.is_grad_enabled()
    return _Fp8Linear.apply(x, weight, bias, module, infer)




def _fused_quant_ready(module) -> bool:
    from ..global_env import global_config
    return (_role(module, "x").scale is not None
            and global_config.fp8_wgrad and torch.is_grad_enabled())


class _Fp8LnLinear(torch.autograd.Function):

    @staticmethod
    def forward(ctx, res, delta, ln_weight, ln_bias, eps, w, bias, module):
        from .. import ops as _ops
        sx = _role(module, "x")
        used = sx.scale.clone()
        h, mean, rstd, xq, xqt, amax = _ops.add_layer_norm_fp8(
            res, delta, ln_weight, ln_bias, eps, used)
        sx.update(amax)
        y, saved = _linear_fwd(ctx, xq, xqt, used, None, w, bias, module,
                               False, res.dtype)
        ctx.has_delta = delta is not None
        if delta is None:
            h = res.contiguous()
        ctx.save_for_backward(*saved, h, ln_weight, mean, rstd)
        out = y.reshape(*res.shape[:-1], w.shape[0])
        return (h, out) if ctx.has_delta else out

    @staticmethod
    def backward(ctx, *grads):
        *lin, h, ln_weight, mean, rstd = ctx.saved_tensors
        dy, dw, db = _linear_bwd(ctx, *lin, grads[-1])
        dy = dy.reshape(h.shape)
        if ctx.has_delta:
            dh = grads[0].contiguous() if grads[0] is not None else None
            dx, dlw, dlb = hip_ops().add_layer_norm_bwd(
                dy, dh, h, ln_weight, mean, rstd)
            g2 = dx
        else:
            dx, dlw, dlb = hip_ops().layer_norm_bwd(dy, h, ln_weight, mean,
                                                    rstd)
            g2 = None
        return (dx, g2, dlw.to(ln_weight.dtype), dlb.to(ln_weight.dtype),
                None, dw, db, None)


def fp8_ln_linear(res: torch.Tensor, delta: Optional[torch.Tensor],
                  ln_weight: torch.Tensor, ln_bias: torch.Tensor, eps: float,
                  weight: torch.Tensor, bias: Optional[torch.Tensor] = None,
                  module=None):
    assert module is not None, "fp8_ln_linear needs the owning module"
    if not _fused_quant_ready(module):
        from .. import ops as _ops
        h, y = _ops.add_layer_norm(res, delta, ln_weight, ln_bias, eps)
        return h, fp8_linear(y, weight, bias, module=module)
    if delta is None:
        return res, _Fp8LnLinear.apply(res, None, ln_weight, ln_bias, eps,
                                       weight, bias, module)
    return _Fp8LnLinear.apply(res, delta, ln_weight, ln_bias, eps, weight,
                              bias, module)


class _Fp8GeluLinear(torch.autograd.Function):

    @staticmethod
    def forward(ctx, x_pre, gelu_bias, w, module):
        from .. import ops as _ops
        shape = x_pre.shape
        x2 = x_pre.reshape(-1, shape[-1]).contiguous()
        sx = _role(module, "x")
        used = sx.scale.clone()
        xq, xqt, amax = _ops.bias_gelu_fp8(x2, gelu_bias, used)
        sx.update(amax)
        y, saved = _linear_fwd(ctx, xq, xqt, used, None, w, None, module,
                               False, x_pre.dtype)
        ctx.save_for_backward(*saved, x2, gelu_bias)
        return y.reshape(*shape[:-1], w.shape[0])

    @staticmethod
    def backward(ctx, dout):
        *lin, x2, gelu_bias = ctx.saved_tensors
        dy, dw, _ = _linear_bwd(ctx, *lin, dout)
        dx, db = hip_ops().bias_gelu_bwd(dy.contiguous(), x2, gelu_bias)
        return (dx.reshape(*dout.shape[:-1], x2.shape[-1]),
                db.to(gelu_bias.dtype), dw, None)


def fp8_gelu_linear(x_pre: torch.Tensor, gelu_bias: torch.Tensor,
                    weight: torch.Tensor, module=None) -> torch.Tensor:
    assert module is not None, "fp8_gelu_linear needs the owning module"
    if not _fused_quant_ready(module):
        from .. import ops as _ops
        return fp8_linear(_ops.bias_gelu(x_pre, gelu_bias), weight,
                          module=module)
    return _Fp8GeluLinear.apply(x_pre, gelu_bias, weight, module)
```

alpa_amd/version.py:

```python
from __future__ import annotations

__version__ = "0.1.0"

MIN_HIP_OPS_ABI = 8


def check_hip_ops_version() -> int:
    from .ops._backend import hip_ops_available, hip_ops
    if not hip_ops_available():
        return -1
    ext = hip_ops()
    abi = getattr(ext, "ABI_VERSION", 0)
    if abi < MIN_HIP_OPS_ABI:
        raise RuntimeError(
            f"alpa_amd HIP extension ABI {abi} < required "
            f"{MIN_HIP_OPS_ABI}: the in-tree _hip_ops.so is stale. "
            "Rebuild it with `python setup.py build_ext --inplace`.")
    return abi
```

Measured before the change: 932.1 TFLOPS.

## Fuse backward reductions for layernorm, bias-GELU and colsum with custom finalize kernel

Layer-norm backward for H up to a limit now computes dx and the dw/db partial sums in one row-striped kernel rather than a per-row dx kernel plus a separate dw/db kernel. Bias-GELU backward folds the bias-gradient partial sum into the dx pass instead of re-reading dx. The partial sums are reduced by a custom finalize kernel that writes the parameter dtype directly, replacing at::sum_out plus .to() casts. This cuts kernel launches and memory passes in the backward pass, at the cost of fewer blocks per kernel and a changed floating-point summation order.

```diff
diff --git a/alpa_amd/ops/__init__.py b/alpa_amd/ops/__init__.py
--- a/alpa_amd/ops/__init__.py
+++ b/alpa_amd/ops/__init__.py
@@ -39,10 +39,11 @@
         x, weight, mean, rstd = ctx.saved_tensors
         if use_hip(x):
             dx, dw, db = hip_ops().layer_norm_bwd(dy.contiguous(), x, weight,
-                                                  mean, rstd)
+                                                  mean, rstd, weight.dtype)
         else:
             dx, dw, db = ref.layer_norm_bwd(dy, x, weight, mean, rstd)
-        return dx, dw.to(weight.dtype), db.to(weight.dtype), None
+            dw, db = dw.to(weight.dtype), db.to(weight.dtype)
+        return dx, dw, db, None
 
 
 def layer_norm(x: torch.Tensor, weight: torch.Tensor, bias: torch.Tensor,
@@ -72,14 +73,15 @@
         dy = dy.contiguous()
         dhc = dh.contiguous() if dh is not None else None
         if use_hip(h):
-            dx, dw, db = hip_ops().add_layer_norm_bwd(dy, dhc, h, weight,
-                                                      mean, rstd)
+            dx, dw, db = hip_ops().add_layer_norm_bwd(
+                dy, dhc, h, weight, mean, rstd, weight.dtype)
         else:
             dx, dw, db = ref.layer_norm_bwd(dy, h, weight, mean, rstd)
+            dw, db = dw.to(weight.dtype), db.to(weight.dtype)
             if dhc is not None:
                 dx = dx + dhc
         g2 = dx if ctx.has_delta else None
-        return dx, g2, dw.to(weight.dtype), db.to(weight.dtype), None
+        return dx, g2, dw, db, None
 
 
 def add_layer_norm(a: torch.Tensor, delta, weight: torch.Tensor,
@@ -103,10 +105,12 @@
     def backward(ctx, dy):
         x, bias = ctx.saved_tensors
         if use_hip(x):
-            dx, db = hip_ops().bias_gelu_bwd(dy.contiguous(), x, bias)
+            dx, db = hip_ops().bias_gelu_bwd(dy.contiguous(), x, bias,
+                                             bias.dtype)
         else:
             dx, db = ref.bias_gelu_bwd(dy, x, bias)
-        return dx, db.to(bias.dtype)
+            db = db.to(bias.dtype)
+        return dx, db
 
 
 def bias_gelu(x: torch.Tensor, bias: torch.Tensor) -> torch.Tensor:
@@ -135,6 +139,12 @@
     return ref.add_layer_norm_fp8(a, delta, weight, bias, eps, scale)
 
 
+def _colsum(g2: torch.Tensor, dtype: torch.dtype) -> torch.Tensor:
+    if dtype in (torch.bfloat16, torch.float32):
+        return hip_ops().colsum_bf16(g2, dtype)
+    return hip_ops().colsum_bf16(g2).to(dtype)
+
+
 class _BiasAdd(torch.autograd.Function):
 
     @staticmethod
@@ -146,9 +156,8 @@
     @staticmethod
     def backward(ctx, g):
         if use_hip(g) and g.dtype == torch.bfloat16:
-            db = hip_ops().colsum_bf16(
-                g.contiguous().reshape(-1, ctx.feat))
-            db = db.to(ctx.bias_dtype)
+            db = _colsum(g.contiguous().reshape(-1, ctx.feat),
+                         ctx.bias_dtype)
         else:
             dims = tuple(range(g.dim() - 1))
             db = g.sum(dim=dims).to(ctx.bias_dtype)
@@ -177,7 +186,7 @@
         dx = (g2 @ w).reshape(*g.shape[:-1], w.shape[1])
         dw = g2.t() @ x2
         if use_hip(g2) and g2.dtype == torch.bfloat16:
-            db = hip_ops().colsum_bf16(g2).to(ctx.bias_dtype)
+            db = _colsum(g2, ctx.bias_dtype)
         else:
             db = g2.sum(0).to(ctx.bias_dtype)
         return dx, dw, db
diff --git a/alpa_amd/ops/csrc/bias_gelu.hip b/alpa_amd/ops/csrc/bias_gelu.hip
--- a/alpa_amd/ops/csrc/bias_gelu.hip
+++ b/alpa_amd/ops/csrc/bias_gelu.hip
@@ -4,10 +4,13 @@
 
 __device__ __forceinline__ float gelu_grad_f(float x) {
   const float k = 0.7978845608028654f;
-  float x2 = x * x;
   float sg = gelu_sigmoid(x);
-  return sg + 2.0f * x * sg * (1.0f - sg) * k *
-                  (1.0f + 3.f * 0.044715f * x2);
+  {
+#pragma clang fp contract(off)
+    float a = 2.0f * x * sg * (1.0f - sg) * k;
+    float p = __builtin_fmaf(x * x, 3.f * 0.044715f, 1.0f);
+    return __builtin_fmaf(p, a, sg);
+  }
 }
 
 __global__ void bias_gelu_fwd_kernel(const short* __restrict__ x,
@@ -26,24 +29,63 @@
   }
 }
 
-__global__ void bias_gelu_bwd_dx_kernel(const short* __restrict__ dy,
-                                        const short* __restrict__ x,
-                                        const short* __restrict__ bias,
-                                        short* __restrict__ dx, int64_t total,
-                                        int F) {
-  int64_t idx = ((int64_t)blockIdx.x * blockDim.x + threadIdx.x) * 8;
-  int64_t stride = (int64_t)gridDim.x * blockDim.x * 8;
-  for (; idx < total; idx += stride) {
-    bf16x8 dv = *reinterpret_cast<const bf16x8*>(dy + idx);
-    bf16x8 xv = *reinterpret_cast<const bf16x8*>(x + idx);
-    bf16x8 bv = *reinterpret_cast<const bf16x8*>(bias + (idx % F));
-    bf16x8 o;
-#pragma unroll
-    for (int j = 0; j < 8; ++j) {
-      float z = bf2f(xv[j]) + bf2f(bv[j]);
-      o[j] = f2bf(bf2f(dv[j]) * gelu_grad_f(z));
-    }
-    *reinterpret_cast<bf16x8*>(dx + idx) = o;
+#define BGB_ROWS 2
+
+__device__ __forceinline__ void bias_gelu_bwd_row(bf16x8 dv, bf16x8 xv,
+                                                  bf16x8 bv, short* dxp,
+                                                  float* s) {
+  bf16x8 o;
+#pragma unroll
+  for (int j = 0; j < 8; ++j) {
+    float z = bf2f(xv[j]) + bf2f(bv[j]);
+    o[j] = f2bf(bf2f(dv[j]) * gelu_grad_f(z));
+    s[j] += bf2f(o[j]);
+  }
+  *reinterpret_cast<bf16x8*>(dxp) = o;
+}
+
+__global__ void __launch_bounds__(256)
+bias_gelu_bwd_kernel(const short* __restrict__ dy, const short* __restrict__ x,
+                     const short* __restrict__ bias, short* __restrict__ dx,
+                     float* __restrict__ db_part, int64_t N, int F) {
+  const int col8 = (blockIdx.x * blockDim.x + threadIdx.x) * 8;
+  const int p = blockIdx.y;
+  const int P = gridDim.y;
+  const int64_t r0 = (int64_t)p * N / P, r1 = (int64_t)(p + 1) * N / P;
+  if (col8 + 8 <= F) {
+    const bf16x8 bv = *reinterpret_cast<const bf16x8*>(bias + col8);
+    float s[8] = {0.f, 0.f, 0.f, 0.f, 0.f, 0.f, 0.f, 0.f};
+    int64_t row = r0;
+    for (; row + BGB_ROWS <= r1; row += BGB_ROWS) {
+      bf16x8 dv[BGB_ROWS], xv[BGB_ROWS];
+#pragma unroll
+      for (int u = 0; u < BGB_ROWS; ++u) {
+        dv[u] = *reinterpret_cast<const bf16x8*>(dy + (row + u) * F + col8);
+        xv[u] = *reinterpret_cast<const bf16x8*>(x + (row + u) * F + col8);
+      }
+#pragma unroll
+      for (int u = 0; u < BGB_ROWS; ++u)
+        bias_gelu_bwd_row(dv[u], xv[u], bv, dx + (row + u) * F + col8, s);
+    }
+    for (; row < r1; ++row) {
+      bf16x8 dv = *reinterpret_cast<const bf16x8*>(dy + row * F + col8);
+      bf16x8 xv = *reinterpret_cast<const bf16x8*>(x + row * F + col8);
+      bias_gelu_bwd_row(dv, xv, bv, dx + row * F + col8, s);
+    }
+#pragma unroll
+    for (int j = 0; j < 8; ++j) db_part[(int64_t)p * F + col8 + j] = s[j];
+  } else if (col8 < F) {
+    for (int c = col8; c < F; ++c) {
+      const float b = bf2f(bias[c]);
+      float s = 0.f;
+      for (int64_t row = r0; row < r1; ++row) {
+        short o = f2bf(bf2f(dy[row * F + c]) *
+                       gelu_grad_f(bf2f(x[row * F + c]) + b));
+        dx[row * F + c] = o;
+        s += bf2f(o);
+      }
+      db_part[(int64_t)p * F + c] = s;
+    }
   }
 }
 
@@ -72,7 +114,62 @@
   }
 }
 
+#define FIN_COLS 32
+#define FIN_SLICES 32
+
+__global__ void __launch_bounds__(FIN_COLS / 4 * FIN_SLICES)
+colsum_finalize_kernel(const float* __restrict__ part_a,
+                       const float* __restrict__ part_b, void* out_a,
+                       void* out_b, int P, int F, int out_bf16) {
+  const float* part = blockIdx.y == 0 ? part_a : part_b;
+  void* out = blockIdx.y == 0 ? out_a : out_b;
+  __shared__ float acc[FIN_SLICES][FIN_COLS];
+  const int quad = threadIdx.x % (FIN_COLS / 4);
+  const int slice = threadIdx.x / (FIN_COLS / 4);
+  const int c0 = blockIdx.x * FIN_COLS + quad * 4;
+  float v[4] = {0.f, 0.f, 0.f, 0.f};
+  if (F % 4 == 0) {
+    if (c0 < F) {
+#pragma unroll 8
+      for (int p = slice; p < P; p += FIN_SLICES) {
+        f32x4 t = *reinterpret_cast<const f32x4*>(part + (int64_t)p * F + c0);
+#pragma unroll
+        for (int k = 0; k < 4; ++k) v[k] += t[k];
+      }
+    }
+  } else {
+    for (int p = slice; p < P; p += FIN_SLICES) {
+#pragma unroll
+      for (int k = 0; k < 4; ++k)
+        if (c0 + k < F) v[k] += part[(int64_t)p * F + c0 + k];
+    }
+  }
+#pragma unroll
+  for (int k = 0; k < 4; ++k) acc[slice][quad * 4 + k] = v[k];
+  __syncthreads();
+  const int c = blockIdx.x * FIN_COLS + threadIdx.x;
+  if (threadIdx.x < FIN_COLS && c < F) {
+    float r = 0.f;
+#pragma unroll
+    for (int s = 0; s < FIN_SLICES; ++s) r += acc[s][threadIdx.x];
+    if (out_bf16)
+      reinterpret_cast<short*>(out)[c] = f2bf(r);
+    else
+      reinterpret_cast<float*>(out)[c] = r;
+  }
+}
+
 extern "C" {
+
+hipError_t launch_colsum_finalize(const float* part_a, const float* part_b,
+                                  void* out_a, void* out_b, int P, int64_t F,
+                                  int out_bf16, hipStream_t stream) {
+  dim3 grid((uint32_t)ceil_div(F, FIN_COLS), part_b != nullptr ? 2 : 1);
+  colsum_finalize_kernel<<<grid, dim3(FIN_COLS / 4 * FIN_SLICES), 0,
+                           stream>>>(part_a, part_b, out_a, out_b, P, (int)F,
+                                     out_bf16);
+  return hipGetLastError();
+}
 
 hipError_t launch_bias_gelu_fwd(const void* x, const void* bias, void* y,
                                 int64_t N, int64_t F, hipStream_t stream) {
@@ -95,15 +192,11 @@
                                 const void* bias, void* dx, float* db_part,
                                 int64_t N, int64_t F, int P,
                                 hipStream_t stream) {
-  int64_t total = N * F;
-  int blocks = (int)min((int64_t)2048, ceil_div(total, 256 * 8));
-  bias_gelu_bwd_dx_kernel<<<dim3(blocks), dim3(256), 0, stream>>>(
+  dim3 grid((uint32_t)ceil_div(F, 256 * 8), P);
+  bias_gelu_bwd_kernel<<<grid, dim3(256), 0, stream>>>(
       (const short*)dy, (const short*)x, (const short*)bias, (short*)dx,
-      total, (int)F);
-  dim3 grid((uint32_t)ceil_div(F, 256 * 8), P);
-  bias_grad_partial_kernel<<<grid, dim3(256), 0, stream>>>(
-      (const short*)dx, db_part, N, (int)F);
-  return hipGetLastError();
-}
-
-}
+      db_part, N, (int)F);
+  return hipGetLastError();
+}
+
+}
diff --git a/alpa_amd/ops/csrc/bindings.cpp b/alpa_amd/ops/csrc/bindings.cpp
--- a/alpa_amd/ops/csrc/bindings.cpp
+++ b/alpa_amd/ops/csrc/bindings.cpp
@@ -105,10 +105,28 @@
   return dims;
 }
 
-int stripes_for(int64_t N, int64_t cols, int64_t chunk_cols) {
-  int64_t chunks = std::max<int64_t>(1, cols / chunk_cols);
+int stripes_for(int64_t N, int64_t cols) {
+  int64_t chunks = std::max<int64_t>(1, cols / 2048);
   int64_t p = std::max<int64_t>(64, 2048 / chunks);
   return (int)std::min<int64_t>({p, N, 512});
+}
+
+at::ScalarType check_out_dtype(const c10::optional<at::ScalarType>& dtype) {
+  const at::ScalarType t = dtype.value_or(at::kFloat);
+  TORCH_CHECK(t == at::kFloat || t == at::kBFloat16,
+              "out_dtype must be fp32 or bf16, got ", dtype_name(t));
+  return t;
+}
+
+void colsum_finalize(const at::Tensor& part, const at::Tensor* part_b,
+                     at::Tensor& out, at::Tensor* out_b) {
+  HIP_OK(launch_colsum_finalize(
+      (const float*)part.const_data_ptr(),
+      part_b != nullptr ? (const float*)part_b->const_data_ptr() : nullptr,
+      out.mutable_data_ptr(),
+      out_b != nullptr ? out_b->mutable_data_ptr() : nullptr,
+      (int)part.size(0), part.size(1),
+      out.scalar_type() == at::kBFloat16 ? 1 : 0, cur_stream()));
 }
 
 
@@ -130,45 +148,42 @@
   return {y, mean, rstd};
 }
 
-std::pair<at::Tensor, at::Tensor> layer_norm_dwdb(const at::Tensor& dy,
-                                                  const at::Tensor& x,
-                                                  const at::Tensor& mean,
-                                                  const at::Tensor& rstd,
-                                                  int64_t N, int64_t H) {
-  auto f32 = x.options().dtype(at::kFloat);
-  auto dw = at::empty({H}, f32);
-  auto db = at::empty({H}, f32);
-  const int kStripes = stripes_for(N, H, 256);
-  auto dw_part = at::empty({kStripes, H}, f32);
-  auto db_part = at::empty({kStripes, H}, f32);
-  HIP_OK(launch_layer_norm_bwd_dwdb(
-      dy.const_data_ptr(), x.const_data_ptr(),
-      (const float*)mean.const_data_ptr(),
-      (const float*)rstd.const_data_ptr(),
-      (float*)dw_part.mutable_data_ptr(), (float*)db_part.mutable_data_ptr(),
-      N, H, kStripes, cur_stream()));
-  at::sum_out(dw, dw_part, {0});
-  at::sum_out(db, db_part, {0});
-  return {dw, db};
-}
-
-std::vector<at::Tensor> layer_norm_bwd(const at::Tensor& dy,
-                                       const at::Tensor& x,
-                                       const at::Tensor& w,
-                                       const at::Tensor& mean,
-                                       const at::Tensor& rstd) {
-  auto [N, H] = check_rows(x, "x", 8, x);
-  check_like(dy, "dy", x, "x");
+std::vector<at::Tensor> layer_norm_bwd_common(
+    const at::Tensor& dy, const at::Tensor* dh, const at::Tensor& x,
+    const char* x_name, const at::Tensor& w, const at::Tensor& mean,
+    const at::Tensor& rstd, const c10::optional<at::ScalarType>& out_dtype) {
+  auto [N, H] = check_rows(x, x_name, 8, x);
+  check_like(dy, "dy", x, x_name);
+  if (dh != nullptr) check_like(*dh, "dh", x, x_name);
   check_vec(w, "w", at::kBFloat16, H, x);
   check_vec(mean, "mean", at::kFloat, N, x);
   check_vec(rstd, "rstd", at::kFloat, N, x);
+  const at::ScalarType odt = check_out_dtype(out_dtype);
+  auto f32 = x.options().dtype(at::kFloat);
   auto dx = at::empty_like(x);
-  HIP_OK(launch_layer_norm_bwd_dx(
-      dy.const_data_ptr(), nullptr, x.const_data_ptr(), w.const_data_ptr(),
-      (const float*)mean.const_data_ptr(), (const float*)rstd.const_data_ptr(),
-      dx.mutable_data_ptr(), N, H, cur_stream()));
-  auto [dw, db] = layer_norm_dwdb(dy, x, mean, rstd, N, H);
+  auto dw = at::empty({H}, x.options().dtype(odt));
+  auto db = at::empty({H}, x.options().dtype(odt));
+  const int kStripes = layer_norm_bwd_stripes(N, H);
+  auto dw_part = at::empty({kStripes, H}, f32);
+  auto db_part = at::empty({kStripes, H}, f32);
+  if (N > 0) {
+    HIP_OK(launch_layer_norm_bwd(
+        dy.const_data_ptr(), dh != nullptr ? dh->const_data_ptr() : nullptr,
+        x.const_data_ptr(), w.const_data_ptr(),
+        (const float*)mean.const_data_ptr(),
+        (const float*)rstd.const_data_ptr(), dx.mutable_data_ptr(),
+        (float*)dw_part.mutable_data_ptr(),
+        (float*)db_part.mutable_data_ptr(), N, H, cur_stream()));
+  }
+  colsum_finalize(dw_part, &db_part, dw, &db);
   return {dx, dw, db};
+}
+
+std::vector<at::Tensor> layer_norm_bwd(
+    const at::Tensor& dy, const at::Tensor& x, const at::Tensor& w,
+    const at::Tensor& mean, const at::Tensor& rstd,
+    const c10::optional<at::ScalarType>& out_dtype) {
+  return layer_norm_bwd_common(dy, nullptr, x, "x", w, mean, rstd, out_dtype);
 }
 
 
@@ -198,22 +213,9 @@
 std::vector<at::Tensor> add_layer_norm_bwd(
     const at::Tensor& dy, const c10::optional<at::Tensor>& dh,
     const at::Tensor& h, const at::Tensor& w, const at::Tensor& mean,
-    const at::Tensor& rstd) {
-  auto [N, H] = check_rows(h, "h", 8, h);
-  check_like(dy, "dy", h, "h");
-  if (dh.has_value()) check_like(*dh, "dh", h, "h");
-  check_vec(w, "w", at::kBFloat16, H, h);
-  check_vec(mean, "mean", at::kFloat, N, h);
-  check_vec(rstd, "rstd", at::kFloat, N, h);
-  auto dx = at::empty_like(h);
-  const void* dhp = dh.has_value() ? dh->const_data_ptr() : nullptr;
-  HIP_OK(launch_layer_norm_bwd_dx(
-      dy.const_data_ptr(), dhp, h.const_data_ptr(), w.const_data_ptr(),
-      (const float*)mean.const_data_ptr(),
-      (const float*)rstd.const_data_ptr(), dx.mutable_data_ptr(), N, H,
-      cur_stream()));
-  auto [dw, db] = layer_norm_dwdb(dy, h, mean, rstd, N, H);
-  return {dx, dw, db};
+    const at::Tensor& rstd, const c10::optional<at::ScalarType>& out_dtype) {
+  return layer_norm_bwd_common(dy, dh.has_value() ? &*dh : nullptr, h, "h", w,
+                               mean, rstd, out_dtype);
 }
 
 
@@ -226,35 +228,40 @@
   return y;
 }
 
-std::vector<at::Tensor> bias_gelu_bwd(const at::Tensor& dy,
-                                      const at::Tensor& x,
-                                      const at::Tensor& bias) {
+std::vector<at::Tensor> bias_gelu_bwd(
+    const at::Tensor& dy, const at::Tensor& x, const at::Tensor& bias,
+    const c10::optional<at::ScalarType>& out_dtype) {
   auto [N, F] = check_rows(x, "x", 8, x);
   check_like(dy, "dy", x, "x");
   check_vec(bias, "bias", at::kBFloat16, F, x);
+  const at::ScalarType odt = check_out_dtype(out_dtype);
   auto dx = at::empty_like(x);
-  auto f32 = x.options().dtype(at::kFloat);
-  const int kStripes = stripes_for(N, F, 2048);
-  auto db = at::empty({F}, f32);
-  auto db_part = at::empty({kStripes, F}, f32);
-  HIP_OK(launch_bias_gelu_bwd(dy.const_data_ptr(), x.const_data_ptr(),
-                              bias.const_data_ptr(), dx.mutable_data_ptr(),
-                              (float*)db_part.mutable_data_ptr(), N, F,
-                              kStripes, cur_stream()));
-  at::sum_out(db, db_part, {0});
+  const int kStripes = stripes_for(N, F);
+  auto db = at::empty({F}, x.options().dtype(odt));
+  auto db_part = at::empty({kStripes, F}, x.options().dtype(at::kFloat));
+  if (N > 0) {
+    HIP_OK(launch_bias_gelu_bwd(dy.const_data_ptr(), x.const_data_ptr(),
+                                bias.const_data_ptr(), dx.mutable_data_ptr(),
+                                (float*)db_part.mutable_data_ptr(), N, F,
+                                kStripes, cur_stream()));
+  }
+  colsum_finalize(db_part, nullptr, db, nullptr);
   return {dx, db};
 }
 
-at::Tensor colsum_bf16(const at::Tensor& t) {
+at::Tensor colsum_bf16(const at::Tensor& t,
+                       const c10::optional<at::ScalarType>& out_dtype) {
   auto [N, F] = check_rows(t, "t", 1, t);
-  auto f32 = t.options().dtype(at::kFloat);
-  const int kStripes = stripes_for(N, F, 2048);
-  auto part = at::empty({kStripes, F}, f32);
-  auto out = at::empty({F}, f32);
-  HIP_OK(launch_colsum_partial(t.const_data_ptr(),
-                               (float*)part.mutable_data_ptr(), N, F,
-                               kStripes, cur_stream()));
-  at::sum_out(out, part, {0});
+  const at::ScalarType odt = check_out_dtype(out_dtype);
+  const int kStripes = stripes_for(N, F);
+  auto part = at::empty({kStripes, F}, t.options().dtype(at::kFloat));
+  auto out = at::empty({F}, t.options().dtype(odt));
+  if (N > 0) {
+    HIP_OK(launch_colsum_partial(t.const_data_ptr(),
+                                 (float*)part.mutable_data_ptr(), N, F,
+                                 kStripes, cur_stream()));
+  }
+  colsum_finalize(part, nullptr, out, nullptr);
   return out;
 }
 
@@ -899,16 +906,23 @@
 }
 
 PYBIND11_MODULE(TORCH_EXTENSION_NAME, m) {
-  m.attr("ABI_VERSION") = 8;
+  m.attr("ABI_VERSION") = 9;
   m.def("layer_norm_fwd", &layer_norm_fwd, "LayerNorm forward (gfx950)");
-  m.def("layer_norm_bwd", &layer_norm_bwd, "LayerNorm backward (gfx950)");
+  m.def("layer_norm_bwd", &layer_norm_bwd, "LayerNorm backward (gfx950)",
+        py::arg("dy"), py::arg("x"), py::arg("w"), py::arg("mean"),
+        py::arg("rstd"), py::arg("out_dtype") = py::none());
   m.def("add_layer_norm_fwd", &add_layer_norm_fwd,
         "fused residual-add + LayerNorm fwd (gfx950)");
   m.def("add_layer_norm_bwd", &add_layer_norm_bwd,
-        "fused residual-add + LayerNorm bwd (gfx950)");
+        "fused residual-add + LayerNorm bwd (gfx950)", py::arg("dy"),
+        py::arg("dh"), py::arg("h"), py::arg("w"), py::arg("mean"),
+        py::arg("rstd"), py::arg("out_dtype") = py::none());
   m.def("bias_gelu_fwd", &bias_gelu_fwd, "bias+GeLU forward (gfx950)");
-  m.def("bias_gelu_bwd", &bias_gelu_bwd, "bias+GeLU backward (gfx950)");
-  m.def("colsum_bf16", &colsum_bf16, "striped column sum (gfx950)");
+  m.def("bias_gelu_bwd", &bias_gelu_bwd, "bias+GeLU backward (gfx950)",
+        py::arg("dy"), py::arg("x"), py::arg("bias"),
+        py::arg("out_dtype") = py::none());
+  m.def("colsum_bf16", &colsum_bf16, "striped column sum (gfx950)",
+        py::arg("t"), py::arg("out_dtype") = py::none());
   m.def("skinny_gemm", &skinny_gemm,
         "decode GEMV over packed weights (gfx950)");
   m.def("adamw_step_raw", &adamw_step_raw, "multi-tensor AdamW (gfx950)",
diff --git a/alpa_amd/ops/csrc/launchers.h b/alpa_amd/ops/csrc/launchers.h
--- a/alpa_amd/ops/csrc/launchers.h
+++ b/alpa_amd/ops/csrc/launchers.h
@@ -9,16 +9,12 @@
 hipError_t launch_layer_norm_fwd(const void* x, const void* w, const void* b,
                                  void* y, float* mean, float* rstd, int64_t N,
                                  int64_t H, float eps, hipStream_t stream);
-hipError_t launch_layer_norm_bwd_dx(const void* dy, const void* dh,
-                                    const void* x, const void* w,
-                                    const float* mean, const float* rstd,
-                                    void* dx, int64_t N, int64_t H,
-                                    hipStream_t stream);
-hipError_t launch_layer_norm_bwd_dwdb(const void* dy, const void* x,
-                                      const float* mean, const float* rstd,
-                                      float* dw_part, float* db_part,
-                                      int64_t N, int64_t H, int P,
-                                      hipStream_t stream);
+int layer_norm_bwd_stripes(int64_t N, int64_t H);
+hipError_t launch_layer_norm_bwd(const void* dy, const void* dh,
+                                 const void* x, const void* w,
+                                 const float* mean, const float* rstd,
+                                 void* dx, float* dw_part, float* db_part,
+                                 int64_t N, int64_t H, hipStream_t stream);
 hipError_t launch_add_layer_norm_fwd(const void* a, const void* b,
                                      const void* w, const void* bias,
                                      void* h, void* y, float* mean,
@@ -33,6 +29,9 @@
                                 hipStream_t stream);
 hipError_t launch_colsum_partial(const void* t, float* part, int64_t N,
                                  int64_t F, int P, hipStream_t stream);
+hipError_t launch_colsum_finalize(const float* part_a, const float* part_b,
+                                  void* out_a, void* out_b, int P, int64_t F,
+                                  int out_bf16, hipStream_t stream);
 
 hipError_t launch_adamw(const void* descs_dev, const void* chunks_dev,
                         int num_chunks, float lr, float beta1, float beta2,
diff --git a/alpa_amd/ops/csrc/layernorm.hip b/alpa_amd/ops/csrc/layernorm.hip
--- a/alpa_amd/ops/csrc/layernorm.hip
+++ b/alpa_amd/ops/csrc/layernorm.hip
@@ -80,6 +80,119 @@
       o[j] = f2bf(g);
     }
     *reinterpret_cast<bf16x8*>(dxr + i) = o;
+  }
+}
+
+#define LNF_MAX_H 4096
+#define LNF_STRIPES 1024
+#define LNF_ROWS 1
+
+template <int RI, bool HAS_DH, int TRIPS>
+__device__ __forceinline__ void layer_norm_bwd_fused_rows(
+    const short* __restrict__ dy, const short* __restrict__ dh,
+    const short* __restrict__ x, const float* __restrict__ mean_in,
+    const float* __restrict__ rstd_in, short* __restrict__ dx,
+    const bf16x8 (&wv)[TRIPS], float (&dw)[TRIPS][8], float (&db)[TRIPS][8],
+    float* red, int64_t row, int H) {
+  bf16x8 dv[RI][TRIPS], xv[RI][TRIPS], hv[RI][TRIPS];
+  float mean[RI], rstd[RI];
+#pragma unroll
+  for (int u = 0; u < RI; ++u) {
+    mean[u] = mean_in[row + u];
+    rstd[u] = rstd_in[row + u];
+#pragma unroll
+    for (int t = 0; t < TRIPS; ++t) {
+      const int i = (t * LN_BLOCK + threadIdx.x) * 8;
+      if (i < H) {
+        const int64_t at = (row + u) * H + i;
+        dv[u][t] = *reinterpret_cast<const bf16x8*>(dy + at);
+        xv[u][t] = *reinterpret_cast<const bf16x8*>(x + at);
+        if (HAS_DH) hv[u][t] = *reinterpret_cast<const bf16x8*>(dh + at);
+      }
+    }
+  }
+#pragma unroll
+  for (int u = 0; u < RI; ++u) {
+    float c1 = 0.f, c2 = 0.f;
+#pragma unroll
+    for (int t = 0; t < TRIPS; ++t) {
+      if ((t * LN_BLOCK + threadIdx.x) * 8 < H) {
+#pragma unroll
+        for (int j = 0; j < 8; ++j) {
+          float wdy = bf2f(dv[u][t][j]) * bf2f(wv[t][j]);
+          float xhat = (bf2f(xv[u][t][j]) - mean[u]) * rstd[u];
+          c1 += wdy;
+          c2 += wdy * xhat;
+        }
+      }
+    }
+    c1 = block_reduce_sum(c1, red) / H;
+    c2 = block_reduce_sum(c2, red) / H;
+#pragma unroll
+    for (int t = 0; t < TRIPS; ++t) {
+      const int i = (t * LN_BLOCK + threadIdx.x) * 8;
+      if (i < H) {
+        bf16x8 o;
+#pragma unroll
+        for (int j = 0; j < 8; ++j) {
+          float d = bf2f(dv[u][t][j]);
+          float wdy = d * bf2f(wv[t][j]);
+          float xhat = (bf2f(xv[u][t][j]) - mean[u]) * rstd[u];
+          float g = (wdy - c1 - xhat * c2) * rstd[u];
+          if (HAS_DH) g += bf2f(hv[u][t][j]);
+          o[j] = f2bf(g);
+          dw[t][j] += d * xhat;
+          db[t][j] += d;
+        }
+        *reinterpret_cast<bf16x8*>(dx + (row + u) * H + i) = o;
+      }
+    }
+  }
+}
+
+template <bool HAS_DH, int TRIPS>
+__global__ void __launch_bounds__(LN_BLOCK)
+layer_norm_bwd_fused_kernel(const short* __restrict__ dy,
+                            const short* __restrict__ dh,
+                            const short* __restrict__ x,
+                            const short* __restrict__ w,
+                            const float* __restrict__ mean_in,
+                            const float* __restrict__ rstd_in,
+                            short* __restrict__ dx,
+                            float* __restrict__ dw_part,
+                            float* __restrict__ db_part, int64_t N, int H) {
+  __shared__ float red[LN_BLOCK / 64];
+  const int p = blockIdx.x;
+  const int P = gridDim.x;
+  const int64_t r0 = (int64_t)p * N / P, r1 = (int64_t)(p + 1) * N / P;
+  bf16x8 wv[TRIPS];
+  float dw[TRIPS][8], db[TRIPS][8];
+#pragma unroll
+  for (int t = 0; t < TRIPS; ++t) {
+    const int i = (t * LN_BLOCK + threadIdx.x) * 8;
+    if (i < H) wv[t] = *reinterpret_cast<const bf16x8*>(w + i);
+#pragma unroll
+    for (int j = 0; j < 8; ++j) dw[t][j] = db[t][j] = 0.f;
+  }
+  int64_t row = r0;
+  for (; row + LNF_ROWS <= r1; row += LNF_ROWS)
+    layer_norm_bwd_fused_rows<LNF_ROWS, HAS_DH, TRIPS>(
+        dy, dh, x, mean_in, rstd_in, dx, wv, dw, db, red, row, H);
+  for (; row < r1; ++row)
+    layer_norm_bwd_fused_rows<1, HAS_DH, TRIPS>(
+        dy, dh, x, mean_in, rstd_in, dx, wv, dw, db, red, row, H);
+#pragma unroll
+  for (int t = 0; t < TRIPS; ++t) {
+    const int i = (t * LN_BLOCK + threadIdx.x) * 8;
+    if (i < H) {
+      float* dwp = dw_part + (int64_t)p * H + i;
+      float* dbp = db_part + (int64_t)p * H + i;
+#pragma unroll
+      for (int j = 0; j < 8; ++j) {
+        dwp[j] = dw[t][j];
+        dbp[j] = db[t][j];
+      }
+    }
   }
 }
 
@@ -140,24 +253,36 @@
   return hipGetLastError();
 }
 
-hipError_t launch_layer_norm_bwd_dx(const void* dy, const void* dh,
-                                    const void* x, const void* w,
-                                    const float* mean, const float* rstd,
-                                    void* dx, int64_t N, int64_t H,
-                                    hipStream_t stream) {
-  auto kernel = dh != nullptr ? layer_norm_bwd_dx_kernel<true>
-                              : layer_norm_bwd_dx_kernel<false>;
-  kernel<<<dim3((uint32_t)N), dim3(LN_BLOCK), 0, stream>>>(
+int layer_norm_bwd_stripes(int64_t N, int64_t H) {
+  if (H <= LNF_MAX_H) return (int)min((int64_t)LNF_STRIPES, N);
+  const int64_t p = max((int64_t)64, 2048 / (H / 256));
+  return (int)min(min(p, N), (int64_t)512);
+}
+
+hipError_t launch_layer_norm_bwd(const void* dy, const void* dh,
+                                 const void* x, const void* w,
+                                 const float* mean, const float* rstd,
+                                 void* dx, float* dw_part, float* db_part,
+                                 int64_t N, int64_t H, hipStream_t stream) {
+  const int P = layer_norm_bwd_stripes(N, H);
+  if (H <= LNF_MAX_H) {
+    const bool one_trip = H <= LN_BLOCK * 8;
+    auto kernel =
+        dh != nullptr
+            ? (one_trip ? layer_norm_bwd_fused_kernel<true, 1>
+                        : layer_norm_bwd_fused_kernel<true, 2>)
+            : (one_trip ? layer_norm_bwd_fused_kernel<false, 1>
+                        : layer_norm_bwd_fused_kernel<false, 2>);
+    kernel<<<dim3(P), dim3(LN_BLOCK), 0, stream>>>(
+        (const short*)dy, (const short*)dh, (const short*)x, (const short*)w,
+        mean, rstd, (short*)dx, dw_part, db_part, N, (int)H);
+    return hipGetLastError();
+  }
+  auto dx_kernel = dh != nullptr ? layer_norm_bwd_dx_kernel<true>
+                                 : layer_norm_bwd_dx_kernel<false>;
+  dx_kernel<<<dim3((uint32_t)N), dim3(LN_BLOCK), 0, stream>>>(
       (const short*)dy, (const short*)dh, (const short*)x, (const short*)w,
       mean, rstd, (short*)dx, (int)H);
-  return hipGetLastError();
-}
-
-hipError_t launch_layer_norm_bwd_dwdb(const void* dy, const void* x,
-                                      const float* mean, const float* rstd,
-                                      float* dw_part, float* db_part,
-                                      int64_t N, int64_t H, int P,
-                                      hipStream_t stream) {
   dim3 grid((uint32_t)ceil_div(H, LNB_COLS * 4), P);
   layer_norm_bwd_dwdb_partial<<<grid, dim3(LNB_COLS), 0, stream>>>(
       (const short*)dy, (const short*)x, mean, rstd, dw_part, db_part,
diff --git a/alpa_amd/ops/fp8.py b/alpa_amd/ops/fp8.py
--- a/alpa_amd/ops/fp8.py
+++ b/alpa_amd/ops/fp8.py
@@ -111,7 +111,7 @@
         dw = dy2.t() @ xsaved
     db = None
     if ctx.has_bias:
-        db = hip_ops().colsum_bf16(dy2).to(dy.dtype)
+        db = hip_ops().colsum_bf16(dy2, dy.dtype)
     return dx, dw, db
 
 
@@ -180,14 +180,13 @@
         if ctx.has_delta:
             dh = grads[0].contiguous() if grads[0] is not None else None
             dx, dlw, dlb = hip_ops().add_layer_norm_bwd(
-                dy, dh, h, ln_weight, mean, rstd)
+                dy, dh, h, ln_weight, mean, rstd, ln_weight.dtype)
             g2 = dx
         else:
             dx, dlw, dlb = hip_ops().layer_norm_bwd(dy, h, ln_weight, mean,
-                                                    rstd)
+                                                    rstd, ln_weight.dtype)
             g2 = None
-        return (dx, g2, dlw.to(ln_weight.dtype), dlb.to(ln_weight.dtype),
-                None, dw, db, None)
+        return (dx, g2, dlw, dlb, None, dw, db, None)
 
 
 def fp8_ln_linear(res: torch.Tensor, delta: Optional[torch.Tensor],
@@ -226,9 +225,9 @@
     def backward(ctx, dout):
         *lin, x2, gelu_bias = ctx.saved_tensors
         dy, dw, _ = _linear_bwd(ctx, *lin, dout)
-        dx, db = hip_ops().bias_gelu_bwd(dy.contiguous(), x2, gelu_bias)
-        return (dx.reshape(*dout.shape[:-1], x2.shape[-1]),
-                db.to(gelu_bias.dtype), dw, None)
+        dx, db = hip_ops().bias_gelu_bwd(dy.contiguous(), x2, gelu_bias,
+                                         gelu_bias.dtype)
+        return (dx.reshape(*dout.shape[:-1], x2.shape[-1]), db, dw, None)
 
 
 def fp8_gelu_linear(x_pre: torch.Tensor, gelu_bias: torch.Tensor,
diff --git a/alpa_amd/version.py b/alpa_amd/version.py
--- a/alpa_amd/version.py
+++ b/alpa_amd/version.py
@@ -2,7 +2,7 @@
 
 __version__ = "0.1.0"
 
-MIN_HIP_OPS_ABI = 8
+MIN_HIP_OPS_ABI = 9
 
 
 def check_hip_ops_version() -> int:
```

Measured after the change: 954.2 TFLOPS (median of 6 runs). 2.4% higher.
